# VodLM/vod

Measured on AMD Instinct MI355X. Metric: queries/sec brute-force top-k (10Mx768 fp16), higher is better.
Workload: dtype f16; 1 GPU; 10000000 sections x 768 f16, batch 1024 queries, top-100, exact brute force; rows_per_gpu=10000000, parallelism=single GPU, engine=ranks, recovery_passes=0

## Files before the change

### include/vodhip.h

```cpp
#ifndef VODHIP_H
#define VODHIP_H

#include <stdint.h>

#ifdef __cplusplus
extern "C" {
#endif

#define VODHIP_VERSION 1

enum { VODHIP_F16 = 0, VODHIP_BF16 = 1, VODHIP_F32 = 2 };
#define VODHIP_EXACT_F32 0x100
#define VODHIP_L2 0x200
enum { VODHIP_HOST = 0, VODHIP_DEVICE = 1 };

typedef struct vodhip_index vodhip_index_t;

const char* vodhip_last_error(void);
int vodhip_version(void);

int vodhip_index_create(int device, int64_t dim, int store_dtype ,
                        int64_t capacity_rows, vodhip_index_t** out);
int vodhip_index_destroy(vodhip_index_t* index);

// ... 16 lines not shown
                              int64_t id_base, float* out_scores, int64_t* out_ids, void* stream);
int vodhip_index_search_finish(vodhip_index_t* index, void* stream);

#define VODHIP_MAX_LISTED 8192
int vodhip_index_score_ids(vodhip_index_t* index, const void* queries, int q_dtype, int64_t nq, const int64_t* ids_dev, int64_t m,
                           int64_t id_base, const int32_t* q_labels_dev , int n_per_query,
                           float* out_scores, void* stream);
int vodhip_index_search_ids(vodhip_index_t* index, const void* queries, int q_dtype, int64_t nq, const int64_t* ids_dev, int64_t m,
                            int k, int64_t id_base, const int32_t* q_labels_dev, int n_per_query, float* out_scores,
                            int64_t* out_ids, void* stream);

#define VODHIP_SUM_IDS_TEMP_BYTES (256ll << 20)
int vodhip_index_sum_ids(vodhip_index_t* index, const int64_t* ids_dev, const float* weights_dev, int64_t nq, int64_t m, int64_t id_base,
                         const int32_t* q_labels_dev , int n_per_query, float* out ,
                         void* stream);

int vodhip_index_log_partition(vodhip_index_t* index, const void* queries, int q_dtype, int64_t nq, float beta,
                               const int32_t* q_labels_dev , int n_per_query,
                               float* out_max , float* out_log_rel , void* stream);

#define VODHIP_POSTERIOR_GROUP_ROWS 16384
#define VODHIP_POSTERIOR_TEMP_BYTES (256ll << 20)
int vodhip_index_posterior_mean(vodhip_index_t* index, const void* queries, int q_dtype, int64_t nq, float beta,
                                const int32_t* q_labels_dev , int n_per_query,
                                float* out_max , float* out_log_rel ,
                                float* out_mean , void* stream);

#define VODHIP_SAMPLE_SLACK_TILES 2
int vodhip_index_sample_posterior(vodhip_index_t* index, const void* queries, int q_dtype, int64_t nq, int k, float beta, uint64_t seed,
                                  int64_t query_offset, int64_t id_base, const int32_t* q_labels_dev ,
                                  int n_per_query, float* out_max , float* out_log_rel ,
                                  int64_t* out_ids , float* out_scores, float* out_log_p,
                                  float* out_log_weight , float* out_keys , void* stream);

#define VODHIP_RANK_MAX_LISTED 64
int vodhip_index_count_above(vodhip_index_t* index, const void* queries, int q_dtype, int64_t nq, const float* thresholds_dev,
                             const int64_t* tie_ids_dev , int64_t m, int64_t id_base,
                             const int32_t* q_labels_dev , int n_per_query,
                             int64_t* out_counts , void* stream);
int vodhip_index_rank_ids(vodhip_index_t* index, const void* queries, int q_dtype, int64_t nq, const int64_t* ids_dev, int64_t m,
                          int64_t id_base, const int32_t* q_labels_dev , int n_per_query,
                          int64_t* out_ranks , float* out_scores , void* stream);
int vodhip_index_scan_score_ids(vodhip_index_t* index, const void* queries, int q_dtype, int64_t nq, const int64_t* ids_dev, int64_t m,
                                int64_t id_base, const int32_t* q_labels_dev , int n_per_query,
                                float* out_scores , int32_t* out_rows , void* stream);

int vodhip_index_set_row_labels(vodhip_index_t* index, const int32_t* labels, int64_t n_rows, int location, void* stream);
int vodhip_index_set_query_labels(vodhip_index_t* index, const int32_t* q_labels_dev, int n_per_query);

int vodhip_index_set_param(vodhip_index_t* index, const char* key, int64_t value);
int vodhip_debug_schedule(int64_t ntotal, int k, int64_t nq, int64_t cand_cap, int64_t dense_rows, int64_t sample_div,
                          int64_t growth_x100, int tile, int recovery_pass, int n_cu, int64_t* out, int max_stages);
int vodhip_index_get_stat(const vodhip_index_t* index, const char* key, int64_t* out);
int vodhip_debug_l2_split(float c, int dtype, uint16_t terms[3], float consts[3]);
int vodhip_debug_tile_order(int64_t ntotal, int64_t* perm_mul, int64_t* perm_mod);
int vodhip_debug_read_probe(int which, int64_t* out, int n);

int vodhip_merge_topk(const float* scores, const int64_t* ids, int n_shards, int64_t nq, int k,
                      int k_out, float* out_scores, int64_t* out_ids, void* stream);
int vodhip_merge_topk_strided(const float* scores, int64_t shard_stride_scores, const int64_t* ids,
                              int64_t shard_stride_ids, int n_shards, int64_t nq, int k, int k_out,
                              float* out_scores, int64_t* out_ids, void* stream);

typedef struct vodhip_node_index vodhip_node_index_t;
int vodhip_node_index_create(int n_devices, const int* devices, int64_t dim, int store_dtype, int64_t capacity_rows,
                             vodhip_node_index_t** out);
int vodhip_node_index_destroy(vodhip_node_index_t* index);
int vodhip_node_index_add(vodhip_node_index_t* index, const void* rows, int64_t n_rows, int src_dtype);
int vodhip_node_index_reset(vodhip_node_index_t* index);
int vodhip_node_index_ntotal(const vodhip_node_index_t* index, int64_t* out);
int vodhip_node_index_n_shards(const vodhip_node_index_t* index);
int vodhip_node_index_shard(vodhip_node_index_t* index, int g, vodhip_index_t** shard, int64_t* id_base, int* device);
int vodhip_node_index_set_param(vodhip_node_index_t* index, const char* key, int64_t value);
int vodhip_node_index_peer_access(const vodhip_node_index_t* index, int* out, int n);
int vodhip_node_index_set_row_labels(vodhip_node_index_t* index, const int32_t* labels, int64_t n_rows);
int vodhip_node_index_set_query_labels(vodhip_node_index_t* index, const int32_t* q_labels, int n_per_query, int location);
int vodhip_node_index_search(vodhip_node_index_t* index, const void* queries, int q_dtype, int64_t nq, int k, int location,
                             float* out_scores, int64_t* out_ids, void* stream);
int vodhip_node_index_search_async(vodhip_node_index_t* index, const void* queries, int q_dtype, int64_t nq, int k, int location,
                                   float* out_scores, int64_t* out_ids, void* stream);
int vodhip_node_index_search_finish(vodhip_node_index_t* index);
int vodhip_node_index_score_ids(vodhip_node_index_t* index, const void* queries, int q_dtype, int64_t nq, const int64_t* ids, int64_t m,
                                const int32_t* q_labels, int n_per_query, int location, float* out_scores, void* stream);
int vodhip_node_index_search_ids(vodhip_node_index_t* index, const void* queries, int q_dtype, int64_t nq, const int64_t* ids, int64_t m,
                                 int k, const int32_t* q_labels, int n_per_query, int location, float* out_scores, int64_t* out_ids,
                                 void* stream);
int vodhip_node_index_sum_ids(vodhip_node_index_t* index, const int64_t* ids, const float* weights, int64_t nq, int64_t m,
                              const int32_t* q_labels, int n_per_query, int location, float* out, void* stream);
int vodhip_node_index_log_partition(vodhip_node_index_t* index, const void* queries, int q_dtype, int64_t nq, float beta,
                                    const int32_t* q_labels , int n_per_query,
                                    float* out_max, float* out_log_rel );
int vodhip_node_index_rank_ids(vodhip_node_index_t* index, const void* queries, int q_dtype, int64_t nq, const int64_t* ids, int64_t m,
                               const int32_t* q_labels , int n_per_query,
                               int64_t* out_ranks, float* out_scores );
int vodhip_node_index_count_above(vodhip_node_index_t* index, const void* queries, int q_dtype, int64_t nq, const float* thresholds,
                                  const int64_t* tie_ids , int64_t m,
                                  const int32_t* q_labels , int n_per_query, int64_t* out_counts );
int vodhip_node_index_posterior_mean(vodhip_node_index_t* index, const void* queries, int q_dtype, int64_t nq, float beta,
                                     const int32_t* q_labels , int n_per_query,
                                     float* out_max, float* out_log_rel , float* out_mean );
int vodhip_node_index_sample_posterior(vodhip_node_index_t* index, const void* queries, int q_dtype, int64_t nq, int k, float beta,
                                       uint64_t seed, int64_t query_offset, const int32_t* q_labels , int n_per_query,
                                       float* out_max, float* out_log_rel , int64_t* out_ids, float* out_scores,
                                       float* out_log_p, float* out_log_weight , float* out_keys );
int vodhip_node_index_get_stat(vodhip_node_index_t* index, const char* key, int64_t* out);

// ... 220 lines not shown
```

### vod_amd/_native.py

```python
from __future__ import annotations

import ctypes
import pathlib
import threading

_LIB_NAME = "libvodhip.so"
_lock = threading.Lock()
_lib: ctypes.CDLL | None = None

F16, BF16, F32 = 0, 1, 2
EXACT_F32 = 0x100
L2 = 0x200
METRICS = {"inner_product": 0, "l2": L2}


def metric_flag(metric: str) -> int:
    if metric not in METRICS:
        raise ValueError(f"metric must be one of {sorted(METRICS)}, got {metric!r}")
    return METRICS[metric]
HOST, DEVICE = 0, 1
MAX_K = 2048
MAX_LISTED = 8192
MAX_ENGINES = 4


class NativeLibraryError(RuntimeError):
    """The HIP extension is missing or a native call failed."""


def lib_path() -> pathlib.Path:
    import os

    override = os.environ.get("VODHIP_LIB")
    if override:
        return pathlib.Path(override)
    return pathlib.Path(__file__).resolve().parent / "csrc" / _LIB_NAME


_c = ctypes
_vp, _i64, _i32, _f32p = _c.c_void_p, _c.c_int64, _c.c_int, _c.c_void_p

SIGNATURES: dict[str, tuple] = {
    "vodhip_last_error": (_c.c_char_p, []),
    "vodhip_version": (_i32, []),
    "vodhip_index_create": (_i32, [_i32, _i64, _i32, _i64, _c.POINTER(_vp)]),
    "vodhip_index_destroy": (_i32, [_vp]),
    "vodhip_index_add": (_i32, [_vp, _vp, _i64, _i32, _i32, _vp]),
    "vodhip_index_reset": (_i32, [_vp]),
    "vodhip_index_ntotal": (_i32, [_vp, _c.POINTER(_i64)]),
    "vodhip_index_dim": (_i32, [_vp, _c.POINTER(_i64)]),
    "vodhip_index_capacity": (_i32, [_vp, _c.POINTER(_i64)]),
    "vodhip_index_data": (_i32, [_vp, _c.POINTER(_vp), _c.POINTER(_i64), _c.POINTER(_i32)]),
    "vodhip_index_get_rows": (_i32, [_vp, _i64, _i64, _vp, _i32, _vp]),
    "vodhip_index_data_f32": (_i32, [_vp, _c.POINTER(_vp), _c.POINTER(_i64)]),
    "vodhip_index_get_rows_f32": (_i32, [_vp, _i64, _i64, _vp, _i32, _vp]),
    "vodhip_index_search": (_i32, [_vp, _vp, _i32, _i64, _i32, _i64, _vp, _vp, _vp]),
    "vodhip_index_search_async": (_i32, [_vp, _vp, _i32, _i64, _i32, _i64, _vp, _vp, _vp]),
    "vodhip_index_search_finish": (_i32, [_vp, _vp]),
    "vodhip_index_score_ids": (_i32, [_vp, _vp, _i32, _i64, _vp, _i64, _i64, _vp, _i32, _vp, _vp]),
    "vodhip_index_search_ids": (_i32, [_vp, _vp, _i32, _i64, _vp, _i64, _i32, _i64, _vp, _i32, _vp, _vp, _vp]),
    "vodhip_index_sum_ids": (_i32, [_vp, _vp, _vp, _i64, _i64, _i64, _vp, _i32, _vp, _vp]),
    "vodhip_index_log_partition": (_i32, [_vp, _vp, _i32, _i64, _c.c_float, _vp, _i32, _vp, _vp, _vp]),
    "vodhip_index_posterior_mean": (_i32, [_vp, _vp, _i32, _i64, _c.c_float, _vp, _i32, _vp, _vp, _vp, _vp]),
    "vodhip_index_count_above": (_i32, [_vp, _vp, _i32, _i64, _vp, _vp, _i64, _i64, _vp, _i32, _vp, _vp]),
    "vodhip_index_rank_ids": (_i32, [_vp, _vp, _i32, _i64, _vp, _i64, _i64, _vp, _i32, _vp, _vp, _vp]),
    "vodhip_index_scan_score_ids": (_i32, [_vp, _vp, _i32, _i64, _vp, _i64, _i64, _vp, _i32, _vp, _vp, _vp]),
    "vodhip_index_sample_posterior": (
        _i32, [_vp, _vp, _i32, _i64, _i32, _c.c_float, _c.c_uint64, _i64, _i64, _vp, _i32, _vp, _vp, _vp, _vp, _vp, _vp, _vp, _vp]),
    "vodhip_index_set_row_labels": (_i32, [_vp, _vp, _i64, _i32, _vp]),
    "vodhip_index_set_query_labels": (_i32, [_vp, _vp, _i32]),
    "vodhip_index_set_param": (_i32, [_vp, _c.c_char_p, _i64]),
    "vodhip_debug_schedule": (_i32, [_i64, _i32, _i64, _i64, _i64, _i64, _i64, _i32, _i32, _i32, _c.POINTER(_i64), _i32]),
    "vodhip_index_get_stat": (_i32, [_vp, _c.c_char_p, _c.POINTER(_i64)]),
    "vodhip_debug_l2_split": (_i32, [_c.c_float, _i32, _c.POINTER(_c.c_uint16), _c.POINTER(_c.c_float)]),
    "vodhip_debug_tile_order": (_i32, [_i64, _c.POINTER(_i64), _c.POINTER(_i64)]),
    "vodhip_debug_read_probe": (_i32, [_i32, _c.POINTER(_i64), _i32]),
    "vodhip_node_index_create": (_i32, [_i32, _c.POINTER(_i32), _i64, _i32, _i64, _c.POINTER(_vp)]),
    "vodhip_node_index_destroy": (_i32, [_vp]),
    "vodhip_node_index_add": (_i32, [_vp, _vp, _i64, _i32]),
    "vodhip_node_index_reset": (_i32, [_vp]),
    "vodhip_node_index_ntotal": (_i32, [_vp, _c.POINTER(_i64)]),
    "vodhip_node_index_n_shards": (_i32, [_vp]),
    "vodhip_node_index_shard": (_i32, [_vp, _i32, _c.POINTER(_vp), _c.POINTER(_i64), _c.POINTER(_i32)]),
    "vodhip_node_index_set_param": (_i32, [_vp, _c.c_char_p, _i64]),
    "vodhip_node_index_get_stat": (_i32, [_vp, _c.c_char_p, _c.POINTER(_i64)]),
    "vodhip_node_index_peer_access": (_i32, [_vp, _c.POINTER(_i32), _i32]),
    "vodhip_node_index_set_row_labels": (_i32, [_vp, _vp, _i64]),
    "vodhip_node_index_set_query_labels": (_i32, [_vp, _vp, _i32, _i32]),
    "vodhip_node_index_search": (_i32, [_vp, _vp, _i32, _i64, _i32, _i32, _vp, _vp, _vp]),
    "vodhip_node_index_search_async": (_i32, [_vp, _vp, _i32, _i64, _i32, _i32, _vp, _vp, _vp]),
    "vodhip_node_index_search_finish": (_i32, [_vp]),
    "vodhip_node_index_score_ids": (_i32, [_vp, _vp, _i32, _i64, _vp, _i64, _vp, _i32, _i32, _vp, _vp]),
    "vodhip_node_index_search_ids": (_i32, [_vp, _vp, _i32, _i64, _vp, _i64, _i32, _vp, _i32, _i32, _vp, _vp, _vp]),
    "vodhip_node_index_sum_ids": (_i32, [_vp, _vp, _vp, _i64, _i64, _vp, _i32, _i32, _vp, _vp]),
    "vodhip_node_index_log_partition": (_i32, [_vp, _vp, _i32, _i64, _c.c_float, _vp, _i32, _vp, _vp]),
    "vodhip_node_index_posterior_mean": (_i32, [_vp, _vp, _i32, _i64, _c.c_float, _vp, _i32, _vp, _vp, _vp]),
    "vodhip_node_index_rank_ids": (_i32, [_vp, _vp, _i32, _i64, _vp, _i64, _vp, _i32, _vp, _vp]),
    "vodhip_node_index_count_above": (_i32, [_vp, _vp, _i32, _i64, _vp, _vp, _i64, _vp, _i32, _vp]),
    "vodhip_node_index_sample_posterior": (
        _i32, [_vp, _vp, _i32, _i64, _i32, _c.c_float, _c.c_uint64, _i64, _vp, _i32, _vp, _vp, _vp, _vp, _vp, _vp, _vp]),
    "vodhip_merge_topk": (_i32, [_vp, _vp, _i32, _i64, _i32, _i32, _vp, _vp, _vp]),
    "vodhip_merge_topk_strided": (_i32, [_vp, _i64, _vp, _i64, _i32, _i64, _i32, _i32, _vp, _vp, _vp]),
    "vodhip_merge_hybrid": (
        _i32,
        [_vp, _vp, _i32, _i32, _c.POINTER(_vp), _c.POINTER(_vp), _c.POINTER(_i32), _c.POINTER(_c.c_float), _i64,
         _vp, _vp, _vp, _c.POINTER(_vp), _i32, _vp, _vp, _vp],
    ),
    "vodhip_retrieval_forward": (
        _i32, [_vp, _vp, _i32, _i32, _i64, _i64, _i64, _vp, _vp, _vp, _vp, _vp, _vp, _vp, _vp, _vp, _vp],
    ),
    "vodhip_retrieval_forward_aux": (
        _i32, [_vp, _vp, _i32, _i32, _i64, _i64, _i64, _vp, _vp, _vp, _vp, _i32, _c.c_float, _c.c_float, _c.c_float,
               _vp, _vp, _vp, _vp, _vp, _vp, _vp, _i64, _vp],
    ),
    "vodhip_retrieval_metrics": (_i32, [_vp, _vp, _i64, _i32, _vp, _i32, _vp, _vp, _vp, _i64, _vp]),
    "vodhip_priority_sample": (
        _i32, [_vp, _vp, _vp, _i64, _i32, _i32, _i32, _c.c_float, _i32, _i32, _vp, _vp, _vp, _vp, _vp],
    ),
    "vodhip_priority_sample_merged": (
        _i32, [_vp, _vp, _vp, _i32, _vp, _vp, _i64, _i64, _i32, _i32, _vp, _vp, _i32, _i32, _vp, _i32, _i32, _c.c_float, _i32, _i32,
               _vp, _vp, _vp, _vp, _vp, _vp, _vp, _vp, _vp],
    ),
    "vodhip_priority_sample_proposal": (
        _i32, [_vp, _vp, _vp, _i64, _i32, _i32, _i32, _c.c_float, _i32, _i32, _vp, _vp, _vp, _vp, _vp, _vp, _vp, _vp],
    ),
    "vodhip_priority_sample_merged_proposal": (
# ... 149 lines not shown
```

### vod_amd/csrc/kernels_exact.hip

```cpp
#include <algorithm>

#include "exact_dot.h"
#include "mips_common.h"
#include "wg_sort.h"

namespace vodhip {

namespace {

__device__ __forceinline__ float round_to_store(float f, int store_dtype) {
    float r;
    (void)store_bits(f, store_dtype, &r);
    return r;
}

constexpr int XT = 512;
#ifndef VODHIP_EXACT_NCR
#define VODHIP_EXACT_NCR 4
#endif
constexpr int NCR = VODHIP_EXACT_NCR;

__device__ __forceinline__ void sort_desc_lds(key_t64* keys, int P, int tid) {
    __syncthreads();
    switch (P) {
// ... 299 lines not shown
                default: exact_dot<NCR>(a.plane, a.stride, rows, qs, a.dim_pad, lane, s); break;
            }
            if (lane == 0) {
#pragma unroll
                for (int n = 0; n < NCR; ++n)
                    if (j0 + n < take) kb[KR + j0 + n] = (rows[n] >= 0 && s[n] == s[n]) ? make_key(s[n], (unsigned)rows[n]) : 0ull;
            }
        }
        int P_eff = 64;
        while (P_eff < KR + take) P_eff <<= 1;
        for (int c = KR + take + tid; c < P_eff; c += XT) kb[c] = 0ull;
        sort_desc_lds(kb, P_eff, tid);
        done += take;
    } while (done < n_total);

    const key_t64 kth = kb[k - 1];
    const float s_k = kth ? unflip_f32((unsigned)(kth >> 32)) : -__builtin_inff();
    for (int c = tid; c < k; c += XT) {
        const key_t64 key = kb[c];
        a.out_scores[qo * k + c] = key ? unflip_f32((unsigned)(key >> 32)) : -__builtin_inff();
        a.out_ids[qo * k + c] = key ? a.id_base + (int64_t)(0xFFFFFFFFu - (unsigned)(key & 0xFFFFFFFFull)) : -1;
    }
    __shared__ int need_s;
    if (!cand_mode) {
        if (tid == 0) need_s = 0;
        __syncthreads();
        for (int j = tid; j < a.kx; j += XT)
            if (a.list_i[qo * a.kx + j] >= 0 && a.list_s[qo * a.kx + j] + eps >= s_k) atomicMax(&need_s, j + 1);
        __syncthreads();
    }
    if (tid == 0) {
        if (cand_mode) {
            if (kth) {
                const float t = s_k - eps;
                if (t > a.thr_s[r]) {
                    a.thr_s[r] = t;
                    a.thr_key[r] = (key_t64)flip_f32(t) << 32;
                }
            }
            a.cnt[(size_t)r * CNT_STRIDE] = 0;
            if (lost) {
                atomicOr(a.flag_word, 1u);
                if (a.flag_q) a.flag_q[r] = 1u;
            }
        } else {
            a.eps[qo] = eps;
            const bool full = a.list_i[qo * a.kx + a.kx - 1] >= 0;
            const bool complete = !full || (a.list_s[qo * a.kx + a.kx - 1] + eps < s_k);
            a.flag_q[qo] = complete ? 0u : 1u;
            if (!complete) atomicOr(a.flag_word, 1u);
            if ((unsigned)need_s > __hip_atomic_load(a.flag_word + 1, __ATOMIC_RELAXED, __HIP_MEMORY_SCOPE_AGENT)) atomicMax(a.flag_word + 1, (unsigned)need_s);
        }
    }
}

hipError_t launch_exact_rescore(const ExactArgs& a, int64_t nq, hipStream_t stream) {
    if (nq <= 0) return hipSuccess;
    const int bytes = (int)((size_t)a.dim_pad * sizeof(float) + (size_t)a.P * (sizeof(key_t64) + sizeof(int)));
    if (hipError_t e = allow_dynamic_lds((const void*)exact_rescore_kernel, bytes); e != hipSuccess) return e;
    hipLaunchKernelGGL(exact_rescore_kernel, dim3((unsigned)nq), dim3(XT), bytes, stream, a);
    return hipGetLastError();
}

}
```

### vod_amd/csrc/kernels_l2.hip

```cpp
#include "../../include/vodhip.h"
#include "l2_bias.h"

extern "C" int vodhip_debug_l2_split(float c, int dtype, uint16_t terms[3], float consts[3]) {
    if ((dtype != VODHIP_F16 && dtype != VODHIP_BF16) || !terms || !consts) return -1;
    uint16_t bits[3];
    vodhip::l2_query_consts(dtype, consts, bits);
    return vodhip::l2_split(c, dtype, terms);
}

#if defined(__HIP__)
#include "mips_common.h"

namespace vodhip {

namespace {

template <int DT>
__device__ __forceinline__ float l2_from_bits(uint16_t b) {
    if constexpr (DT == 0) return (float)__builtin_bit_cast(_Float16, b);
    else return __uint_as_float((unsigned int)b << 16);
}

__device__ __forceinline__ float l2_wave_sum(float v) {
#pragma unroll
// ... 10 lines not shown
    uint16_t* x = rows + row * stride;
    float acc = 0.f;
    for (int c0 = lane * 8; c0 < dim; c0 += 64 * 8) {
        const uint4 w = *(const uint4*)(x + c0);
        const unsigned int u[4] = {w.x, w.y, w.z, w.w};
#pragma unroll
        for (int e = 0; e < 8; ++e) {
            const float v = l2_from_bits<DT>((uint16_t)(u[e >> 1] >> ((e & 1) * 16)));
            if (c0 + e < dim) acc = fmaf(v, v, acc);
        }
    }
    const float n2 = l2_wave_sum(acc);
    if (lane == 0) {
        uint16_t t[3];
        if (l2_split(-0.5f * n2, DT, t)) atomicAdd(saturated, 1u);
        x[dim] = t[0];
        x[dim + 1] = t[1];
        x[dim + 2] = t[2];
    }
}

template <int DT>
__global__ void __launch_bounds__(256) l2_stage_queries_kernel(const void* __restrict__ q_src, int q_dtype, int64_t nq, int dim,
                                                               uint16_t* __restrict__ staged, float* __restrict__ qn) {
    const int lane = threadIdx.x & 63;
    const int64_t row = (int64_t)blockIdx.x * 4 + (threadIdx.x >> 6);
    if (row >= nq) return;
    uint16_t* out = staged + row * (int64_t)(dim + L2_BIAS_COLS);
    float acc = 0.f;
    for (int c0 = lane * 8; c0 < dim; c0 += 64 * 8) {
        for (int e = 0; e < 8 && c0 + e < dim; ++e) {
            const int64_t at = row * dim + c0 + e;
            float f;
            if (q_dtype == 2) f = ((const float*)q_src)[at];
            else if (q_dtype == 0) f = (float)(((const _Float16*)q_src)[at]);
            else f = (float)(((const __bf16*)q_src)[at]);
            float v;
            out[c0 + e] = store_bits(f, DT, &v);
            acc = fmaf(v, v, acc);
        }
    }
    const float n2 = l2_wave_sum(acc);
    if (lane == 0) {
        float a[3];
        uint16_t bits[3];
        l2_query_consts(DT, a, bits);
        out[dim] = bits[0];
        out[dim + 1] = bits[1];
        out[dim + 2] = bits[2];
        qn[row] = n2;
    }
}

__global__ void __launch_bounds__(256) l2_finish_kernel(const float* __restrict__ sim, const float* __restrict__ qn, int64_t nq, int k, float* __restrict__ dist) {
    const int64_t i = (int64_t)blockIdx.x * blockDim.x + threadIdx.x;
    if (i >= nq * k) return;
    const float s = sim[i];
    float d = __builtin_inff();
    if (s != -__builtin_inff()) d = fmaxf(0.f, qn[i / k] - 2.f * s);
    dist[i] = d;
}

}

hipError_t launch_l2_bias(void* rows, int store_dtype, int64_t n_rows, int64_t dim, int64_t stride, unsigned int* saturated,
                          hipStream_t stream) {
    if (n_rows == 0) return hipSuccess;
    if (dim + L2_BIAS_COLS > stride || stride % 64 != 0 || dim > (1ll << 30)) return hipErrorInvalidValue;
    const unsigned blocks = (unsigned)((n_rows + 3) / 4);
    if (store_dtype == 0)
        hipLaunchKernelGGL(l2_bias_kernel<0>, dim3(blocks), dim3(256), 0, stream, (uint16_t*)rows, n_rows, (int)dim, stride, saturated);
    else
        hipLaunchKernelGGL(l2_bias_kernel<1>, dim3(blocks), dim3(256), 0, stream, (uint16_t*)rows, n_rows, (int)dim, stride, saturated);
    return hipGetLastError();
}

hipError_t launch_l2_stage_queries(const void* q_src, int q_dtype, int64_t nq, int64_t dim, int store_dtype, void* staged, float* qn,
                                   hipStream_t stream) {
    if (nq == 0) return hipSuccess;
    if (dim > (1ll << 30)) return hipErrorInvalidValue;
    const unsigned blocks = (unsigned)((nq + 3) / 4);
    if (store_dtype == 0)
        hipLaunchKernelGGL(l2_stage_queries_kernel<0>, dim3(blocks), dim3(256), 0, stream, q_src, q_dtype, nq, (int)dim, (uint16_t*)staged, qn);
    else
        hipLaunchKernelGGL(l2_stage_queries_kernel<1>, dim3(blocks), dim3(256), 0, stream, q_src, q_dtype, nq, (int)dim, (uint16_t*)staged, qn);
    return hipGetLastError();
}

hipError_t launch_l2_finish(const float* sim, const float* qn, int64_t nq, int k, float* dist, hipStream_t stream) {
    if (nq == 0) return hipSuccess;
    const int64_t n = nq * k;
    hipLaunchKernelGGL(l2_finish_kernel, dim3((unsigned)((n + 255) / 256)), dim3(256), 0, stream, sim, qn, nq, k, dist);
    return hipGetLastError();
}

}
#endif
```

### vod_amd/csrc/kernels_mips.hip

```cpp
#include "mips_common.h"
#include "wg_sort.h"

#include <algorithm>
#include <cstdlib>
#include <map>
#include <mutex>
#include <utility>
#include <type_traits>

namespace vodhip {

enum : int { MODE_FILTER = 0, MODE_DENSE = 1, MODE_GMAX = 2 };

template <int DT, int BM, int BN, int WM, int WN, int NSTAGE, int MODE, bool SUBSET = false>
__global__ __launch_bounds__(WM* WN * 64, (WM * WN * 64 * ((160 * 1024) / (NSTAGE * (BM + BN) * 128))) / 256 >= 2 ? 2 : 1)
void mips_filter_kernel(
    const uint16_t* __restrict__ X, const uint16_t* __restrict__ Q, int dim_pad, int row_begin, int row_end,
    int n_xtiles, int n_qtiles, int nq, const float* __restrict__ thr_s, const key_t64* __restrict__ thr_key,
    key_t64* __restrict__ cand, unsigned int* __restrict__ cnt, int cap, unsigned int* __restrict__ overflow, FilterExtra ex) {
    constexpr int BK = 64;
    constexpr int NWAVES = WM * WN;
    constexpr int TM = BM / WM, TN = BN / WN;
    constexpr int MI = TM / 32, NJ = TN / 32;
    constexpr int ROW_BYTES = BK * 2;
    constexpr int RPI = 8;
    constexpr int KK = BK / 16;
    constexpr int A_BYTES = BM * ROW_BYTES, B_BYTES = BN * ROW_BYTES;
    constexpr int STAGE_BYTES = A_BYTES + B_BYTES;
    constexpr int NA = BM / RPI / NWAVES;
    constexpr int NB = BN / RPI / NWAVES;
    constexpr int G = NA + NB;
    static_assert(BM % (RPI * NWAVES) == 0 && BN % (RPI * NWAVES) == 0, "tile/wave mismatch");
    static_assert(NSTAGE >= 2 && NSTAGE <= 3, "ring depth");

    extern __shared__ __attribute__((aligned(16))) char smem[];

    const int bid = blockIdx.x;
    const int xcd = bid & 7, jj = bid >> 3;
    const int qt = jj % n_qtiles;
    const int xt = (jj / n_qtiles) * 8 + xcd;
    if (xt >= n_xtiles) return;

    const int tid = threadIdx.x;
    const int lane = tid & 63;
    const int wave = __builtin_amdgcn_readfirstlane(tid >> 6);
    const int wm = wave / WN, wn = wave % WN;

    const int x0 = MODE == MODE_FILTER ? filter_tile_row0(ex, row_begin, xt, BM) : row_begin + xt * BM;
    const int q0 = qt * BN;

    const int st_row = lane >> 3, st_slot = lane & 7;
    const char* a_src[NA];
    const char* b_src[NB];
#pragma unroll
    for (int t = 0; t < NA; ++t) {
        const int r = (wave * NA + t) * RPI + st_row;
        const int c = st_slot ^ ((r >> 1) & 7);
        size_t grow = (size_t)(x0 + r);
        if constexpr (MODE == MODE_GMAX) {
            const int bb = r & 31;
            const int grp_in_tile = ((r / TM) * MI + (r % TM) / 32) * 2 + ((bb >> 2) & 1);
            const int idx = (bb >> 3) * 4 + (bb & 3);
            grow = ((size_t)idx * (size_t)ex.sample_groups + (size_t)xt * (BM / 16) + grp_in_tile) * (size_t)ex.sample_rstride + (size_t)ex.sample_offset;
        }
        a_src[t] = (const char*)X + (grow * dim_pad + c * 8) * 2;
    }
#pragma unroll
    for (int t = 0; t < NB; ++t) {
        const int r = (wave * NB + t) * RPI + st_row;
        const int c = st_slot ^ ((r >> 1) & 7);
        b_src[t] = (const char*)Q + ((size_t)(q0 + r) * dim_pad + c * 8) * 2;
    }
    auto stage_part = [&](int ks, int part, int nparts) {
        char* sa = smem + (ks % NSTAGE) * STAGE_BYTES;
        char* sb = sa + A_BYTES;
        const int kbyte = ks * ROW_BYTES;
#pragma unroll
        for (int u = 0; u < G; ++u) {
            if ((u * nparts) / G != part) continue;
            if (u < NA)
                glds16(a_src[u] + kbyte, sa + (wave * NA + u) * RPI * ROW_BYTES);
            else
                glds16(b_src[u - NA] + kbyte, sb + (wave * NB + (u - NA)) * RPI * ROW_BYTES);
        }
    };

    const int fr = lane & 31, fh = lane >> 5;
    const int swz = (fr >> 1) & 7;
    const int a_row_off = (wm * TM + fr) * ROW_BYTES;
    const int b_row_off = A_BYTES + (wn * TN + fr) * ROW_BYTES;

    f32x16 acc[MI][NJ];
#pragma unroll
    for (int i = 0; i < MI; ++i)
// ... 55 lines not shown
    }
    for (; t < nk; ++t) {
        if (NSTAGE >= 3 && nk - 1 - t >= 1) wait_vmcnt<(NSTAGE >= 3 ? 1 : 0) * G>();
        else wait_vmcnt<0>();
        __builtin_amdgcn_s_barrier();
        kslice(t, std::false_type{});
    }

#pragma unroll
    for (int j = 0; j < NJ; ++j) {
        const int q = q0 + wn * TN + j * 32 + fr;
        const bool q_ok = q < nq;
#pragma unroll
        for (int i = 0; i < MI; ++i) {
            const int rbase = x0 + wm * TM + i * 32 + 4 * fh;
            if constexpr (MODE == MODE_DENSE) {
                if (q_ok) {
#pragma unroll
                    for (int r = 0; r < 16; ++r) {
                        const int row = rbase + (r & 3) + 8 * (r >> 2);
                        const float s = acc[i][j][r];
                        if (row < row_end) {
                            const key_t64 key = (s == s) ? make_key(s, (unsigned)row) : 0ull;
                            cand[(size_t)q * cap + (row - row_begin)] = key;
                        }
                    }
                    if constexpr (SUBSET) {
#pragma unroll 1
                        for (int r = 0; r < 16; ++r) {
                            const int row = rbase + (r & 3) + 8 * (r >> 2);
                            if (row < row_end && !subset_allows(ex, q, row)) cand[(size_t)q * cap + (row - row_begin)] = 0ull;
                        }
                    }
                }
            } else {
                float m = acc[i][j][0];
#pragma unroll
                for (int r = 1; r < 16; ++r) m = fmaxf(m, acc[i][j][r]);
                if constexpr (MODE == MODE_GMAX) {
                    const int slot = xt * (BM / 16) + (wm * MI + i) * 2 + fh;
                    if (q_ok) cand[(size_t)q * cap + slot] = (m == m) ? make_key(m, (unsigned)slot) : 0ull;
                } else {
                    const bool hit = m >= thr[j];
                    if (__any(hit)) {
                        if (hit)
                            append_survivors<16, SUBSET>(
                                thr[j], q, row_end, [&](int r) { return acc[i][j][r]; },
                                [&](int r) { return rbase + (r & 3) + 8 * (r >> 2); }, thr_key, cand, cnt, cap, overflow, ex);
                    }
                }
            }
        }
    }
}

constexpr int WSTG_CAP = 256;
constexpr int WSTG_FLUSH = 176;
constexpr int WSTG_BYTES = 8 * WSTG_CAP * 12;
template <int DT, int MODE, bool SUBSET, bool STAGGER>
__global__ __launch_bounds__(512, 2) void mips_filter16p_kernel(
    const uint16_t* __restrict__ X, const uint16_t* __restrict__ Q, int dim_pad, int row_begin, int row_end,
    int n_xtiles, int n_qtiles, int nq, const float* __restrict__ thr_s, const key_t64* __restrict__ thr_key,
    key_t64* __restrict__ cand, unsigned int* __restrict__ cnt, int cap, unsigned int* __restrict__ overflow, FilterExtra ex) {
    static_assert(MODE == MODE_FILTER || MODE == MODE_GMAX, "dense chunks run on mips_filter_kernel");
    constexpr int BM = 256, BN = 256, WN = 4, NWAVES = 8, BK = 64, NSTAGE = 2;
    constexpr int TM = 128, TN = 64;
    constexpr int MB = TM / 16, NB16 = TN / 16;
    constexpr int ROW_BYTES = BK * 2, RPI = 8;
    constexpr int A_BYTES = BM * ROW_BYTES, STAGE_BYTES = (BM + BN) * ROW_BYTES;
    constexpr int NA = BM / RPI / NWAVES, NBI = BN / RPI / NWAVES, G = NA + NBI;

    extern __shared__ __attribute__((aligned(16))) char smem[];
    const int bid = blockIdx.x;
    const int xcd = bid & 7, jj = bid >> 3;
    const int qt = jj % n_qtiles;
    const int xt0 = (jj / n_qtiles) * 8 + xcd;
    const int xt_step = (int)gridDim.x / n_qtiles;
    if (xt0 >= n_xtiles) return;
    const int n_my = (n_xtiles - 1 - xt0) / xt_step + 1;
    const int tid = threadIdx.x;
    const int lane = tid & 63;
    const int wave = __builtin_amdgcn_readfirstlane(tid >> 6);
    const int wm = wave / WN, wn = wave % WN;
    const int q0 = qt * BN;
    const int nk = dim_pad / BK;
    const size_t tile_rows_stride = MODE == MODE_GMAX ? (size_t)8 * (size_t)ex.sample_rstride : (size_t)BM;
    size_t tile_step_bytes = (size_t)xt_step * tile_rows_stride * dim_pad * 2;
#ifdef VODHIP_ABLATION
    const bool abl_l2hot = (ex.flags & (1 << 8)) != 0;
    const bool abl_dma_early = (ex.flags & (2 << 8)) != 0;
    const bool abl_prio = (ex.flags & (4 << 8)) != 0;
    const bool abl_nosurv = (ex.flags & (8 << 8)) != 0;
    const bool abl_corpus_nt = (ex.flags & (16 << 8)) != 0;
    const bool abl_corpus_sc0 = (ex.flags & (32 << 8)) != 0;
    const bool abl_blocked = (ex.flags & (64 << 8)) != 0;
    const bool abl_q0 = (ex.flags & (128 << 8)) != 0;
    if (abl_l2hot) tile_step_bytes = 0;
    if (abl_prio && wave >= NWAVES / 2) __builtin_amdgcn_s_setprio(1);
#else
    constexpr bool abl_l2hot = false, abl_dma_early = false, abl_nosurv = false, abl_blocked = false, abl_q0 = false;
#endif

    const int st_row = lane >> 3, st_slot = lane & 7;
    const char* a_src[NA];
    const char* b_src[NBI];
#pragma unroll
    for (int t = 0; t < NA; ++t) {
        const int r = (wave * NA + t) * RPI + st_row;
        size_t grow = (size_t)filter_tile_row0(ex, row_begin, abl_l2hot ? (xt0 & 15) : xt0, BM) + r;
        if constexpr (MODE == MODE_GMAX) {
            const int grp_in_tile = (r >> 7) * 4 + ((r >> 2) & 3);
            const int idx = ((r >> 4) & 7) * 4 + (r & 3);
            grow = ((size_t)idx * (size_t)ex.sample_groups + (size_t)xt0 * 8 + grp_in_tile) * (size_t)ex.sample_rstride + (size_t)ex.sample_offset;
        }
        a_src[t] = (const char*)X + (grow * dim_pad + (st_slot ^ ((r >> 1) & 7)) * 8) * 2;
        if (abl_blocked)
            a_src[t] = (const char*)X + ((size_t)row_begin + (size_t)xt0 * BM) * dim_pad * 2 + (size_t)r * ROW_BYTES + (st_slot ^ ((r >> 1) & 7)) * 16;
    }
#pragma unroll
    for (int t = 0; t < NBI; ++t) {
        const int r = (wave * NBI + t) * RPI + st_row;
        b_src[t] = (const char*)Q + ((size_t)((abl_q0 ? 0 : q0) + r) * dim_pad + (st_slot ^ ((r >> 1) & 7)) * 8) * 2;
    }
    const bool corpus_nt = (ex.flags & FILTER_FLAG_CORPUS_NT) != 0;
    auto stage_part = [&](int slot, int kbyte, int part, int nparts) {
        char* sa = smem + slot * STAGE_BYTES;
        char* sb = sa + A_BYTES;
#pragma unroll
        for (int u = 0; u < G; ++u) {
            if ((u * nparts) / G != part) continue;
            if (u < NA) {
// ... 148 lines not shown
        ++g;
    };
    Frags fp;
    bool pre_b = false;
    int kbyte_b = 0;
    auto slice_b_head = [&](int it, int t) {
        wait_vmcnt<0>();
        __builtin_amdgcn_s_barrier();
        next_fetch(it, t, pre_b, kbyte_b);
        if (pre_b) stage_part((g + 1) & 1, kbyte_b, 0, 2);
    };
    auto slice_b_body = [&](auto first_tag) {
        constexpr bool FIRST = decltype(first_tag)::value;
        const char* base = smem + (g & 1) * STAGE_BYTES;
        __builtin_amdgcn_sched_barrier(0);
        Frags f;
        read_b(base, 0, f);
        read_a(base, 0, f, 0, 8);
        if (pre_b) stage_part((g + 1) & 1, kbyte_b, 1, 2);
        __builtin_amdgcn_sched_barrier(0);
        mma(f, 0, 8, FIRST);
        __builtin_amdgcn_sched_barrier(0);
        read_b(base, 1, fp);
        read_a(base, 1, fp, 0, 8);
        asm volatile("s_waitcnt lgkmcnt(0)" ::: "memory");
        __builtin_amdgcn_sched_barrier(0);
        ++g;
    };
    if (!STAGGER || wave < NWAVES / 2) {
        for (int it = 0; it < n_my; ++it) {
            slice_a(it, 0, std::true_type{});
            for (int t = 1; t < nk; ++t) slice_a(it, t, std::false_type{});
            epilogue(xt0 + it * xt_step, tile_row0(it));
        }
    } else {
        for (int it = 0; it <= n_my; ++it) {
            if (it < n_my) slice_b_head(it, 0);
            if (it > 0) {
                mma(fp, 0, 8, false);
                __builtin_amdgcn_sched_barrier(0);
                epilogue(xt0 + (it - 1) * xt_step, tile_row0(it - 1));
            }
            if (it < n_my) {
                slice_b_body(std::true_type{});
                for (int t = 1; t < nk; ++t) {
                    slice_b_head(it, t);
                    mma(fp, 0, 8, false);
                    slice_b_body(std::false_type{});
                }
            }
        }
    }
    if constexpr (MODE == MODE_FILTER) wl.flush(out);
}

__device__ __forceinline__ void bitonic_sort_desc_lds(key_t64* keys, int P, int tid) {
    constexpr int CE_UNROLL = 4;
    const int half = P >> 1;
    for (int size = 2; size <= P; size <<= 1) {
        for (int stride = size >> 1; stride > 0; stride >>= 1) {
            __syncthreads();
            for (int t0 = tid; t0 < half; t0 += 256 * CE_UNROLL) {
                key_t64 a[CE_UNROLL], b[CE_UNROLL];
                int pos[CE_UNROLL];
#pragma unroll
                for (int u = 0; u < CE_UNROLL; ++u) {
                    const int t = t0 + u * 256;
                    pos[u] = 2 * t - (t & (stride - 1));
                    if (t < half) {
                        a[u] = keys[pos[u]];
                        b[u] = keys[pos[u] + stride];
                    }
                }
#pragma unroll
                for (int u = 0; u < CE_UNROLL; ++u) {
                    const int t = t0 + u * 256;
                    if (t < half) {
                        const bool desc = (pos[u] & size) == 0;
                        if ((a[u] < b[u]) == desc) {
                            keys[pos[u]] = b[u];
                            keys[pos[u] + stride] = a[u];
                        }
                    }
                }
            }
        }
    }
    __syncthreads();
}

constexpr int SEL_HIST_INTS = 544;

template <typename Op>
__device__ __forceinline__ int wave_scan_dpp(int v, int identity, Op op) {
    v = op(v, __builtin_amdgcn_update_dpp(identity, v, 0x111, 0xf, 0xf, false));
    v = op(v, __builtin_amdgcn_update_dpp(identity, v, 0x112, 0xf, 0xf, false));
    v = op(v, __builtin_amdgcn_update_dpp(identity, v, 0x114, 0xf, 0xf, false));
    v = op(v, __builtin_amdgcn_update_dpp(identity, v, 0x118, 0xf, 0xf, false));
    v = op(v, __builtin_amdgcn_update_dpp(identity, v, 0x142, 0xa, 0xf, false));
    v = op(v, __builtin_amdgcn_update_dpp(identity, v, 0x143, 0xc, 0xf, false));
    return v;
}
#ifdef VODHIP_ABLATION
__device__ long long g_probe_select[256];
#endif
#define RSEL_PROBE(i) VODHIP_PROBE(g_probe_select, ppb + (i))
// ... 63 lines not shown
                    hist[514] = hh[j];
                }
        }
        __syncthreads();
        if (pass < 4) RSEL_PROBE(2 + 2 * pass);
        const int digit = hist[512];
        rank = hist[513];
        const int in_bin = hist[514];
        prefix |= (key_t64)digit << sh;
        mask |= dmask << sh;
        hi_bit = sh - 1;
        if (in_bin == 1 && hi_bit >= 0) {
#pragma unroll
            for (int u = 0; u < KPT; ++u) {
                const key_t64 e = mine[u];
                if (e != 0ull && (e & mask) == prefix) {
                    hist[515] = (int)(unsigned)(e & 0xFFFFFFFFull);
                    hist[516] = (int)(unsigned)(e >> 32);
                }
            }
            __syncthreads();
            return ((key_t64)(unsigned)hist[516] << 32) | (key_t64)(unsigned)hist[515];
        }
    }
    return prefix;
}

__device__ __forceinline__ void sort_front_desc(key_t64* keys, int kp, int tid) {
    __syncthreads();
    if (kp <= 512) {
        if (tid < 64) {
            switch (kp) {
                case 64: wave_sort_regs<1, true>(keys, tid); break;
                case 128: wave_sort_regs<2, true>(keys, tid); break;
                case 256: wave_sort_regs<4, true>(keys, tid); break;
                default: wave_sort_regs<8, true>(keys, tid); break;
            }
        }
        __syncthreads();
    } else if (!wg_sort_lds_256<true>(keys, kp, tid)) {
        bitonic_sort_desc_lds(keys, kp, tid);
    }
}

enum : int { SELECT_FINAL = 1, SELECT_THRESHOLD_ONLY = 2 };
#define SEL_PROBE(i) VODHIP_PROBE(g_probe_select, pb + (i))
template <int KPT>
__global__ __launch_bounds__(256) void mips_select_kernel(key_t64* __restrict__ topk, int kp, int k,
                                                          const key_t64* __restrict__ cand,
                                                          unsigned int* __restrict__ cnt, int cap, int dense_n,
                                                          float* __restrict__ thr_s, key_t64* __restrict__ thr_key,
                                                          unsigned int* __restrict__ overflow, unsigned int* __restrict__ ovf_q, int flags,
                                                          int64_t id_base, float* __restrict__ out_scores,
                                                          int64_t* __restrict__ out_ids, const int* __restrict__ q_map) {
    extern __shared__ __attribute__((aligned(16))) char smem[];
    int* hist = (int*)smem;
    key_t64* front = (key_t64*)(hist + SEL_HIST_INTS);
    const int q = blockIdx.x;
    const int tid = threadIdx.x;
    const bool final_sort = (flags & SELECT_FINAL) != 0;
    const bool thr_only = (flags & SELECT_THRESHOLD_ONLY) != 0;
    [[maybe_unused]] const int pb = final_sort ? 0 : thr_only ? 8 : 16;
    SEL_PROBE(0);
    key_t64 mine[KPT];
    const key_t64* cq = cand + (size_t)q * cap;
#pragma unroll
    for (int u = 0; u < KPT; ++u) {
        const int i = tid + u * 256;
        if (i < kp) mine[u] = thr_only ? 0ull : topk[(size_t)q * kp + i];
        else mine[u] = (i - kp) < cap ? cq[i - kp] : 0ull;
    }
    unsigned n = dense_n >= 0 ? (unsigned)dense_n : cnt[(size_t)q * CNT_STRIDE];
    if (n > (unsigned)cap) {
        if (tid == 0) {
            atomicOr(overflow, 1u);
            if (ovf_q) ovf_q[q] = 1u;
        }
        n = cap;
    }
    const int room = KPT * 256 - kp;
    int done = 0;
    key_t64 kth = 0;
    do {
        const int take = min((int)n - done, room);
        const int total = kp + take;
        if (done > 0) {
#pragma unroll
            for (int u = 0; u < KPT; ++u) {
                const int i = tid + u * 256;
                mine[u] = i < kp ? front[i] : (i < total ? cq[done + (i - kp)] : 0ull);
            }
        } else {
#pragma unroll
            for (int u = 0; u < KPT; ++u)
                if (tid + u * 256 >= total) mine[u] = 0ull;
        }
        if (tid == 0) hist[517] = 0;
        SEL_PROBE(1);
        kth = radix_select_kth_regs<KPT>(mine, k, hist, tid, 24 + 10 * (pb >> 3));
        SEL_PROBE(2);
        done += take;
        if (!thr_only || done < (int)n) {
            unsigned long long keep[KPT];
            int n_wave = 0;
#pragma unroll
            for (int u = 0; u < KPT; ++u) {
                keep[u] = __ballot(mine[u] >= kth && mine[u] != 0ull);
                n_wave += __builtin_popcountll(keep[u]);
            }
            int base = 0;
            if ((tid & 63) == 0 && n_wave) base = atomicAdd(&hist[517], n_wave);
            base = __builtin_amdgcn_readfirstlane(base);
            const unsigned long long below = (1ull << (tid & 63)) - 1ull;
#pragma unroll
            for (int u = 0; u < KPT; ++u) {
                const int at = base + __builtin_popcountll(keep[u] & below);
                if (((keep[u] >> (tid & 63)) & 1ull) && at < kp) front[at] = mine[u];
                base += __builtin_popcountll(keep[u]);
            }
            __syncthreads();
            const int n_kept = min(hist[517], kp);
            for (int i = n_kept + tid; i < kp; i += 256) front[i] = 0ull;
            __syncthreads();
        }
    } while (done < (int)n);
    SEL_PROBE(3);
    if (final_sort) {
        sort_front_desc(front, kp, tid);
        kth = front[k - 1];
    }
    SEL_PROBE(4);
    if (!thr_only)
        for (int i = tid; i < kp; i += 256) topk[(size_t)q * kp + i] = front[i];
    if (out_scores != nullptr) {
        const size_t qo = q_map ? (size_t)q_map[q] : (size_t)q;
        for (int c = tid; c < k; c += 256) {
            const key_t64 key = front[c];
            out_scores[qo * k + c] = key ? unflip_f32((unsigned)(key >> 32)) : -__builtin_inff();
            out_ids[qo * k + c] = key ? id_base + (int64_t)(0xFFFFFFFFu - (unsigned)(key & 0xFFFFFFFFu)) : -1;
        }
    }
    if (tid == 0) {
        if (thr_only) kth &= 0xFFFFFFFF00000000ull;
        const key_t64 old = thr_key[q];
        if (kth > old) {
            thr_key[q] = kth;
            thr_s[q] = unflip_f32((unsigned)(kth >> 32));
        }
        cnt[(size_t)q * CNT_STRIDE] = 0;
    }
    SEL_PROBE(5);
    if (tid == 0 && q == 0) {
        [[maybe_unused]] const long long nn = (long long)n;
#ifdef VODHIP_ABLATION
        g_probe_select[2 * (pb + 6)] = nn;
        g_probe_select[2 * (pb + 6) + 1] = 1;
#endif
    }
}

__global__ void mips_output_kernel(const key_t64* __restrict__ topk, int kp, int k, int64_t nq, int64_t id_base,
                                   float* __restrict__ out_scores, int64_t* __restrict__ out_ids) {
    const int64_t i = (int64_t)blockIdx.x * blockDim.x + threadIdx.x;
    if (i >= nq * k) return;
    const int64_t q = i / k;
    const int c = (int)(i % k);
    const key_t64 key = topk[q * kp + c];
    if (key == 0) {
        out_scores[i] = -__builtin_inff();
        out_ids[i] = -1;
    } else {
        out_scores[i] = unflip_f32((unsigned)(key >> 32));
        out_ids[i] = id_base + (int64_t)(0xFFFFFFFFu - (unsigned)(key & 0xFFFFFFFFu));
    }
}

template <int SRC, int DST>
__global__ void convert_rows_kernel(const void* __restrict__ src, int64_t n_rows, int64_t dim, uint16_t* __restrict__ dst,
                                    int64_t dst_stride) {
    const int64_t chunks_per_row = dst_stride / 8;
    const int64_t i = (int64_t)blockIdx.x * blockDim.x + threadIdx.x;
    if (i >= n_rows * chunks_per_row) return;
    const int64_t row = i / chunks_per_row;
    const int64_t c0 = (i % chunks_per_row) * 8;
    uint16_t out[8];
#pragma unroll
    for (int e = 0; e < 8; ++e) {
        const int64_t c = c0 + e;
        uint16_t v = 0;
        if (c < dim) {
            float f;
            if constexpr (SRC == 2) {
                f = ((const float*)src)[row * dim + c];
            } else if constexpr (SRC == 0) {
                f = (float)(((const _Float16*)src)[row * dim + c]);
            } else {
                f = (float)(((const __bf16*)src)[row * dim + c]);
            }
            float rounded;
            v = store_bits(f, DST, &rounded);
        }
        out[e] = v;
    }
    *(uint4*)(dst + row * dst_stride + c0) = *(const uint4*)out;
}

hipError_t launch_convert_rows(const void* src, int src_dtype, int64_t n_rows, int64_t dim, void* dst, int dst_dtype,
                               int64_t dst_stride, hipStream_t stream) {
    if (n_rows == 0) return hipSuccess;
    const int64_t total = n_rows * (dst_stride / 8);
    const int threads = 256;
// ... 8 lines not shown
    VOD_CONV(0, 0) VOD_CONV(1, 0) VOD_CONV(2, 0) VOD_CONV(0, 1) VOD_CONV(1, 1) VOD_CONV(2, 1)
#undef VOD_CONV
    return hipErrorInvalidValue;
}

__global__ void mips_prepare_kernel(const void* __restrict__ q_src, int q_dtype, int64_t nq, int64_t dim,
                                    uint16_t* __restrict__ q_pad, int store_dtype, int64_t nq_pad, int64_t dim_pad,
                                    key_t64* __restrict__ topk, int64_t n_topk, unsigned int* __restrict__ cnt,
                                    float* __restrict__ thr_s, key_t64* __restrict__ thr_key,
                                    unsigned int* __restrict__ overflow, unsigned int* __restrict__ ovf_q, int clear_overflow,
                                    const float* __restrict__ seed_scores, const int64_t* __restrict__ seed_ids, int k,
                                    const int* __restrict__ q_map, const float* __restrict__ seed_margin) {
    const int64_t i = (int64_t)blockIdx.x * blockDim.x + threadIdx.x;
    const int64_t chunks_per_row = dim_pad / 8;
    if (i < nq_pad * chunks_per_row) {
        const int64_t row = i / chunks_per_row;
        const int64_t c0 = (i % chunks_per_row) * 8;
        uint16_t out[8];
#pragma unroll
        for (int e = 0; e < 8; ++e) {
            const int64_t c = c0 + e;
            uint16_t v = 0;
            if (row < nq && c < dim) {
                const int64_t srow = q_map ? (int64_t)q_map[row] : row;
                float f;
                if (q_dtype == 2) f = ((const float*)q_src)[srow * dim + c];
                else if (q_dtype == 0) f = (float)(((const _Float16*)q_src)[srow * dim + c]);
                else f = (float)(((const __bf16*)q_src)[srow * dim + c]);
                float rounded;
                v = store_bits(f, store_dtype, &rounded);
            }
            out[e] = v;
        }
        *(uint4*)(q_pad + row * dim_pad + c0) = *(const uint4*)out;
    }
    if (i < n_topk) topk[i] = 0;
    if (i < nq_pad) {
        cnt[i * CNT_STRIDE] = 0;
        float ts = -__builtin_inff();
        key_t64 tk = 0;
        const int64_t srow = (q_map && i < nq) ? (int64_t)q_map[i] : i;
        if (ovf_q != nullptr && i < nq) ovf_q[i] = 0u;
        if (seed_scores != nullptr && i < nq && seed_ids[srow * k + (k - 1)] >= 0) {
            float s = seed_scores[srow * k + (k - 1)];
            if (seed_margin != nullptr) s -= seed_margin[srow];
            if (s == s) {
                ts = s;
                tk = (key_t64)flip_f32(s) << 32;
            }
        }
        thr_s[i] = ts;
        thr_key[i] = tk;
    }
    if (i == 0 && clear_overflow) {
        overflow[0] = 0u;
        overflow[1] = 0u;
        overflow[2] = 0u;
        overflow[3] = 0u;
    }
}

hipError_t launch_search_prepare(const SearchWorkspace& ws, const void* q_src, int q_dtype, int64_t nq, int64_t dim,
                                 int store_dtype, int64_t nq_pad, int64_t dim_pad, bool clear_overflow,
                                 const float* seed_scores, const int64_t* seed_ids, int k, const int* q_map, hipStream_t stream,
                                 const float* seed_margin) {
    const int64_t n_topk = nq_pad * ws.kp;
    const int64_t n = std::max(n_topk, nq_pad * (dim_pad / 8));
    const int threads = 256;
    const unsigned blocks = (unsigned)((n + threads - 1) / threads);
    hipLaunchKernelGGL(mips_prepare_kernel, dim3(blocks), dim3(threads), 0, stream, q_src, q_dtype, nq, dim,
                       (uint16_t*)ws.q_pad, store_dtype, nq_pad, dim_pad, ws.topk, n_topk, ws.cnt, ws.thr_s, ws.thr_key,
                       ws.overflow, ws.ovf_q, clear_overflow ? 1 : 0, seed_scores, seed_ids, k, q_map, seed_margin);
    return hipGetLastError();
}

hipError_t allow_dynamic_lds(const void* kernel, int bytes) {
    static std::mutex mu;
    static std::map<std::pair<int, const void*>, int> granted;
    int dev = 0;
    hipError_t e = hipGetDevice(&dev);
    if (e != hipSuccess) return e;
    std::lock_guard<std::mutex> lock(mu);
    auto it = granted.find({dev, kernel});
    if (it != granted.end() && it->second >= bytes) return hipSuccess;
    e = hipFuncSetAttribute(kernel, hipFuncAttributeMaxDynamicSharedMemorySize, bytes);
    if (e == hipSuccess) granted[{dev, kernel}] = bytes;
    return e;
}

namespace {

struct FilterLaunch {
    const void* store;
    const void* q_pad;
    int64_t dim_pad, row_begin, row_end, nq, nq_pad;
    int n_xtiles;
    const SearchWorkspace* ws;
    hipStream_t stream;
};

template <int DT, int BM, int BN, int WM, int WN, int NSTAGE, int MODE, bool SUBSET>
hipError_t launch_generic(const FilterLaunch& L) {
    const int n_qtiles = (int)(L.nq_pad / BN);
    const unsigned grid = (unsigned)((L.n_xtiles + 7) / 8) * 8u * (unsigned)n_qtiles;
    constexpr int threads = WM * WN * 64;
    constexpr size_t lds = (size_t)NSTAGE * (BM + BN) * 128;
    auto kern = mips_filter_kernel<DT, BM, BN, WM, WN, NSTAGE, MODE, SUBSET>;
// ... 30 lines not shown
    if (hipError_t e = allow_dynamic_lds((const void*)kern, (int)lds); e != hipSuccess) return e;
    const SearchWorkspace& ws = *L.ws;
    hipLaunchKernelGGL(kern, dim3((unsigned)grid), dim3(512), lds, L.stream, (const uint16_t*)L.store, (const uint16_t*)L.q_pad,
                       (int)L.dim_pad, (int)L.row_begin, (int)L.row_end, L.n_xtiles, n_qtiles, (int)L.nq, ws.thr_s, ws.thr_key,
                       ws.cand, ws.cnt, (int)ws.cap, ws.overflow, ws.extra);
    return hipGetLastError();
}

template <int DT, bool STAGGER>
hipError_t launch_persistent_mode(const FilterLaunch& L, int mode, bool subset) {
    constexpr FilterGeometry G = geometry(STAGGER ? FilterKernel::Staggered : FilterKernel::Persistent);
    static_assert(G.rows == 256 && G.cols == 256 && G.group_rows == 32 && G.persistent, "the planner's geometry of mips_filter16p_kernel");
    if (mode == MODE_DENSE) return hipErrorInvalidValue;
    if (mode == MODE_GMAX) return launch_persistent<DT, MODE_GMAX, false, STAGGER>(L);
    return subset ? launch_persistent<DT, MODE_FILTER, true, STAGGER>(L) : launch_persistent<DT, MODE_FILTER, false, STAGGER>(L);
}

template <int DT>
hipError_t launch_filter_dt(FilterKernel kernel, int mode, bool subset, const FilterLaunch& L) {
    switch (kernel) {
        case FilterKernel::Generic128: return launch_generic_mode<DT, FilterKernel::Generic128, 128, 128, 2, 2, 2>(L, mode, subset);
        case FilterKernel::Generic256x64: return launch_generic_mode<DT, FilterKernel::Generic256x64, 256, 64, 4, 1, 3>(L, mode, subset);
        case FilterKernel::Generic256x128: return launch_generic_mode<DT, FilterKernel::Generic256x128, 256, 128, 4, 2, 3>(L, mode, subset);
        case FilterKernel::Persistent: return launch_persistent_mode<DT, false>(L, mode, subset);
        case FilterKernel::Staggered: return launch_persistent_mode<DT, true>(L, mode, subset);
        default: return hipErrorInvalidValue;
    }
}

}

hipError_t launch_filter(int store_dtype, FilterKernel kernel, int mode, const void* store, const void* q_pad, int64_t dim_pad,
                         int64_t row_begin, int64_t row_end, int64_t n_sample_tiles, int64_t nq, int64_t nq_pad,
                         const SearchWorkspace& ws, hipStream_t stream, FilterStageFn experiment) {
    if (mode != MODE_GMAX && row_end <= row_begin) return hipSuccess;
    if (mode == MODE_GMAX && n_sample_tiles <= 0) return hipSuccess;
    if (experiment && mode == MODE_FILTER) return experiment(store_dtype, store, q_pad, dim_pad, row_begin, row_end, nq, nq_pad, ws, stream);
    if (kernel == FilterKernel::EightPhase)
        return mode == MODE_FILTER ? launch_filter_8phase(store_dtype, 7, true, store, q_pad, dim_pad, row_begin, row_end, nq, nq_pad, ws, stream)
                                   : hipErrorInvalidValue;
    const int bm = geometry(kernel).rows;
    int n_xtiles = mode == MODE_GMAX ? (int)n_sample_tiles : (int)((row_end - row_begin + bm - 1) / bm);
    if (mode == MODE_FILTER && ws.extra.perm_mod > 0) {
        n_xtiles = (int)((row_end - row_begin + 255) / 256) * (256 / bm);
        row_end = ws.extra.row_bound;
    }
    FilterLaunch L{store, q_pad, dim_pad, row_begin, row_end, nq, nq_pad, n_xtiles, &ws, stream};
    const bool subset = ws.extra.row_label != nullptr;
    return store_dtype == 0 ? launch_filter_dt<0>(kernel, mode, subset, L) : launch_filter_dt<1>(kernel, mode, subset, L);
}

template <int KPT>
static hipError_t launch_select_kpt(const SearchWorkspace& ws, int64_t nq, int k, int64_t dense_n, int flags, hipStream_t stream,
                                    int64_t id_base, float* out_scores, int64_t* out_ids, const int* q_map) {
    const size_t lds = SEL_HIST_INTS * sizeof(int) + (size_t)ws.kp * sizeof(key_t64);
    const bool final_sort = (flags & SELECT_FINAL) != 0;
    hipLaunchKernelGGL(mips_select_kernel<KPT>, dim3((unsigned)nq), dim3(256), lds, stream, ws.topk, (int)ws.kp, k, ws.cand,
                       ws.cnt, (int)ws.cap, (int)dense_n, ws.thr_s, ws.thr_key, ws.overflow, ws.ovf_q, flags, id_base,
                       final_sort ? out_scores : nullptr, final_sort ? out_ids : nullptr, q_map);
    return hipGetLastError();
}

hipError_t launch_select(const SearchWorkspace& ws, int64_t nq, int k, int64_t dense_n, int flags, hipStream_t stream,
                         int64_t id_base, float* out_scores, int64_t* out_ids, const int* q_map) {
    int sb = 2048;
    while (sb < 2 * ws.kp) sb <<= 1;
    while (dense_n > sb - ws.kp && sb < 8192) sb <<= 1;
    switch (sb) {
        case 2048: return launch_select_kpt<8>(ws, nq, k, dense_n, flags, stream, id_base, out_scores, out_ids, q_map);
        case 4096: return launch_select_kpt<16>(ws, nq, k, dense_n, flags, stream, id_base, out_scores, out_ids, q_map);
        default: return launch_select_kpt<32>(ws, nq, k, dense_n, flags, stream, id_base, out_scores, out_ids, q_map);
    }
}

hipError_t launch_output(const SearchWorkspace& ws, int64_t nq, int k, int64_t id_base, float* out_scores,
                         int64_t* out_ids, hipStream_t stream) {
    const int64_t total = nq * k;
    if (total == 0) return hipSuccess;
    const unsigned blocks = (unsigned)((total + 255) / 256);
    hipLaunchKernelGGL(mips_output_kernel, dim3(blocks), dim3(256), 0, stream, ws.topk, (int)ws.kp, k, nq, id_base,
                       out_scores, out_ids);
    return hipGetLastError();
}

__device__ __forceinline__ bool pair_before(float sa, int64_t ia, float sb, int64_t ib) {
    const bool va = ia >= 0, vb = ib >= 0;
    if (va != vb) return va;
    if (!va) return false;
    if (sa != sb) return sa > sb;
    return ia < ib;
}

__device__ __forceinline__ void merge_ce(float* ssc, int64_t* sid, int a, int b) {
    const float sa = ssc[a], sb = ssc[b];
    const int64_t ia = sid[a], ib = sid[b];
    if (pair_before(sb, ib, sa, ia)) {
        ssc[a] = sb;
        ssc[b] = sa;
        sid[a] = ib;
        sid[b] = ia;
    }
}

__global__ __launch_bounds__(256) void merge_topk_kernel(const float* __restrict__ scores, const int64_t* __restrict__ ids,
                                                         int64_t stride_s, int64_t stride_i, int n_shards, int64_t nq, int k, int k_out,
                                                         int L, int S2, int flat, float* __restrict__ out_scores,
                                                         int64_t* __restrict__ out_ids) {
    extern __shared__ __attribute__((aligned(16))) char smem[];
    const int P = S2 * L;
    int64_t* sid = (int64_t*)smem;
    float* ssc = (float*)(smem + (size_t)P * 8);
    int* s_flag = (int*)(smem + (size_t)P * 12);
    const int64_t q = blockIdx.x;
    const int tid = threadIdx.x;
    const int lmask = L - 1, lshift = 31 - __builtin_clz(L);
    if (tid == 0) *s_flag = 0;
    for (int i = tid; i < P; i += 256) {
        const int t = flat ? i / k : i >> lshift, c = flat ? i % k : i & lmask;
        float s = -__builtin_inff();
        int64_t id = -1;
        if (t < n_shards && c < k) {
            s = scores[(int64_t)t * stride_s + q * k + c];
            id = ids[(int64_t)t * stride_i + q * k + c];
            if (id < 0 || s != s) {
// ... 88 lines not shown
```

### vod_amd/csrc/kernels_mips_8phase.hip

```cpp
#include <hip/hip_runtime.h>

#include <type_traits>

#include "mips_common.h"

namespace vodhip {

namespace {
constexpr int P8_HALF = 128 * 128;
constexpr int P8_OPERANDS = 8 * P8_HALF;
constexpr int P8_WL_CAP = 256;
constexpr int P8_WL_FLUSH = 176;
constexpr int P8_TRANSPOSE_MAX_LANES = 2;
constexpr int P8_XPOSE = 8 * 2 * 32 * 4;
constexpr int P8_DRAIN_RECORDS = 112;
constexpr int P8_SC1 = 16;
static_assert(P8_DRAIN_RECORDS % 8 == 0 && P8_DRAIN_RECORDS * 132 + 256 <= P8_OPERANDS / 8, "drain staging");
constexpr int P8_LDS = P8_OPERANDS + 8 * P8_WL_CAP * 12 + P8_XPOSE;
static_assert(P8_LDS <= 160 * 1024, "LDS budget");
}

template <int DT, bool SUBSET, bool KEEPB0, int LEAD = 7>
__global__ __launch_bounds__(512, 2) void mips_filter8ph_kernel(
    const uint16_t* __restrict__ X, const uint16_t* __restrict__ Q, int dim_pad, int row_begin, int row_end, int n_xtiles,
    int n_qtiles, int nq, const float* __restrict__ thr_s, const key_t64* __restrict__ thr_key, key_t64* __restrict__ cand,
    unsigned int* __restrict__ cnt, int cap, unsigned int* __restrict__ overflow, FilterExtra ex, float* __restrict__ ring, int ring_cap) {
    constexpr int BM = 256, BN = 256, WN = 4, NWAVES = 8, TM = 128, TN = 64, MB = TM / 16, NB16 = TN / 16, ROW_BYTES = 128;
    extern __shared__ __attribute__((aligned(16))) char smem[];
    const int bid = blockIdx.x;
    const int xcd = bid & 7, jj = bid >> 3;
    const int qt = jj % n_qtiles;
    const int xt0 = (jj / n_qtiles) * 8 + xcd;
    const int xt_step = (int)gridDim.x / n_qtiles;
    if (xt0 >= n_xtiles) return;
    const int n_my = (n_xtiles - 1 - xt0) / xt_step + 1;
    const int tid = threadIdx.x;
    const int lane = tid & 63;
    const int wave = __builtin_amdgcn_readfirstlane(tid >> 6);
    const int wm = wave / WN, wn = wave % WN;
    const int q0 = qt * BN;
    const int nk = dim_pad / 64;
    const size_t row_stride = (size_t)dim_pad * 2;

    const int st_row = lane >> 3, st_slot = lane & 7;
    int super_cur = ex.perm_mod > 0 ? filter_tile_row0(ex, row_begin, xt0, BM) / BM : 0;
    int super_epi = super_cur;
    const int perm_inc = ex.perm_mod > 0 ? (int)(((unsigned long long)xt_step * (unsigned long long)ex.perm_mul) % (unsigned long long)ex.perm_mod) : 0;
    const char* a_src[2];
    const char* b_src[2];
#pragma unroll
    for (int u = 0; u < 2; ++u) {
        const int sw = (u * 4 + (st_row >> 1)) & 7;
        const int arow = (wave >> 2) * 128 + (wave & 3) * 16 + u * 8 + st_row;
        const int brow = (wave >> 1) * 64 + (wave & 1) * 16 + u * 8 + st_row;
        a_src[u] = (const char*)X + ((size_t)filter_tile_row0(ex, row_begin, xt0, BM) + arow) * row_stride + ((st_slot ^ sw) << 4);
#ifdef VODHIP_ABLATION
        const int q0_stage = (ex.flags & (128 << 8)) ? 0 : q0;
#else
        const int q0_stage = q0;
#endif
        b_src[u] = (const char*)Q + (size_t)(q0_stage + brow) * row_stride + ((st_slot ^ sw) << 4);
    }
    const size_t a_half_step = 64 * row_stride, b_half_step = 32 * row_stride;
    const size_t tile_step_bytes = (size_t)xt_step * BM * row_stride;

    const bool corpus_nt = (ex.flags & FILTER_FLAG_CORPUS_NT) != 0;
    int s_t = 0, s_it = 0, s_par = 0;
    int issued = 0;
    bool s_active = n_my > 0;
    auto stage = [&](auto kind_tag) {
        constexpr int KIND = decltype(kind_tag)::value;
        if (s_active) {
            char* dst = smem + (s_par * 4 + KIND) * P8_HALF + wave * 16 * ROW_BYTES;
            const int kbyte = s_t * ROW_BYTES;
            if constexpr (KIND == 0 || KIND == 2) {
                const size_t off = (KIND == 2 ? a_half_step : 0) + kbyte;
                if (corpus_nt) {
                    glds16_aux<2>(a_src[0] + off, dst);
                    glds16_aux<2>(a_src[1] + off, dst + 8 * ROW_BYTES);
                } else {
                    glds16(a_src[0] + off, dst);
                    glds16(a_src[1] + off, dst + 8 * ROW_BYTES);
                }
            } else if constexpr (KIND == 1) {
                glds16(b_src[0] + b_half_step + kbyte, dst);
                glds16(b_src[1] + b_half_step + kbyte, dst + 8 * ROW_BYTES);
            } else {
                glds16(b_src[0] + kbyte, dst);
                glds16(b_src[1] + kbyte, dst + 8 * ROW_BYTES);
            }
            ++issued;
            if constexpr (KIND == 3) {
                s_par ^= 1;
                if (++s_t == nk) {
                    s_t = 0;
                    ++s_it;
                    if (s_it < n_my) {
                        long long step = (long long)tile_step_bytes;
                        if (ex.perm_mod > 0) {
                            int nxt = super_cur + perm_inc;
                            if (nxt >= ex.perm_mod) nxt -= ex.perm_mod;
                            step = (long long)(nxt - super_cur) * (long long)BM * (long long)row_stride;
                            super_cur = nxt;
                        }
                        a_src[0] += step;
                        a_src[1] += step;
                    } else {
                        s_active = false;
                    }
                }
            }
        }
    };
    using K0 = std::integral_constant<int, 0>;
    using K1 = std::integral_constant<int, 1>;
    using K2 = std::integral_constant<int, 2>;
    using K3 = std::integral_constant<int, 3>;

    const int fr = lane & 15, fq = lane >> 4;
    const int swz = (fr >> 1) & 7;

    float thr[NB16];
#pragma unroll
    for (int j = 0; j < NB16; ++j) {
        const int q = q0 + wn * TN + j * 16 + fr;
        thr[j] = q < nq ? thr_s[q] : __builtin_inff();
    }
#pragma unroll
    for (int j = 0; j < NB16; ++j) asm volatile("" : "+v"(thr[j]));
    wait_vmcnt<0>();

    WaveSurvivorList<P8_WL_CAP, SUBSET> wl(smem + P8_OPERANDS, NWAVES, wave);
    const SurvivorOut out{thr_key, cand, cnt, cap, overflow, ex};
    auto wl_append = [&](bool p, key_t64 key, int q) { if (wl.append(p, key, q, out)) wait_vmcnt<0>(); };
    auto wl_flush = [&]() { wl.flush(out); wait_vmcnt<0>(); };
    float* const xpose = (float*)(smem + P8_OPERANDS + NWAVES * P8_WL_CAP * 12) + wave * 64;
    const size_t ring_wave = (size_t)bid * NWAVES + wave;
    float* const ring_w = ring + ring_wave * ring_cap * 32;
    unsigned* const ring_meta = (unsigned*)(ring + (size_t)gridDim.x * NWAVES * ring_cap * 32) + ring_wave * ring_cap;
    int ring_n = 0;
    int ring_fallbacks = 0;

    f32x4 acc[MB][NB16];
    u32x4 fa[4], fb[2], fa1[4], fb1[2];
    u32x4 fc[2], fc1[2];
#ifdef P8_KNOBS
    const bool knob_no_stagger = (ex.flags & (1 << 8)) != 0, knob_no_prio = (ex.flags & (2 << 8)) != 0;
#else
    constexpr bool knob_no_stagger = false, knob_no_prio = false;
#endif

    auto read_a = [&](const char* half) {
        const char* base = half + (wm * 64 + fr) * ROW_BYTES;
        const int s0 = ((0 + fq) ^ swz) << 4, s1 = ((4 + fq) ^ swz) << 4;
#pragma unroll
        for (int i = 0; i < 4; ++i) {
            fa[i] = *(const u32x4*)(base + i * 16 * ROW_BYTES + s0);
            fa1[i] = *(const u32x4*)(base + i * 16 * ROW_BYTES + s1);
        }
    };
    auto read_b = [&](const char* half) {
        const char* base = half + (wn * 32 + fr) * ROW_BYTES;
        const int s0 = ((0 + fq) ^ swz) << 4, s1 = ((4 + fq) ^ swz) << 4;
#pragma unroll
        for (int j = 0; j < 2; ++j) {
            fb[j] = *(const u32x4*)(base + j * 16 * ROW_BYTES + s0);
            fb1[j] = *(const u32x4*)(base + j * 16 * ROW_BYTES + s1);
        }
    };
    auto read_b1 = [&](const char* half) {
        const char* base = half + (wn * 32 + fr) * ROW_BYTES;
        const int s0 = ((0 + fq) ^ swz) << 4, s1 = ((4 + fq) ^ swz) << 4;
#pragma unroll
        for (int j = 0; j < 2; ++j) {
            if constexpr (KEEPB0) {
                fc[j] = *(const u32x4*)(base + j * 16 * ROW_BYTES + s0);
                fc1[j] = *(const u32x4*)(base + j * 16 * ROW_BYTES + s1);
            } else {
                fb[j] = *(const u32x4*)(base + j * 16 * ROW_BYTES + s0);
                fb1[j] = *(const u32x4*)(base + j * 16 * ROW_BYTES + s1);
            }
        }
    };
// ... 198 lines not shown
        if (ex.perm_mod > 0) {
            int nxt = super_epi + perm_inc;
            if (nxt >= ex.perm_mod) nxt -= ex.perm_mod;
            super_epi = nxt;
        }
    }
    if (wm == 0 && !knob_no_stagger) __builtin_amdgcn_s_barrier();

#ifndef P8_ABL_NO_DRAIN
    if (ring_n > 0) {
        wait_vmcnt<0>();
        if (fq == 0) {
#pragma unroll
            for (int j = 0; j < NB16; ++j) xpose[j * 16 + fr] = thr[j];
        }
        wave_lds_exchange();
        char* const stage_w = smem + wave * (P8_OPERANDS / NWAVES);
        const float* const sums = (const float*)stage_w;
        const unsigned* const meta = (const unsigned*)(stage_w + P8_DRAIN_RECORDS * 128);
        const int half = lane >> 5, t = lane & 31;
        for (int r0 = 0; r0 < ring_n; r0 += P8_DRAIN_RECORDS) {
#pragma unroll
            for (int i = 0; i < P8_DRAIN_RECORDS / 8; ++i) {
                const int r = min(r0 + i * 8 + (lane >> 3), ring_n - 1);
                __builtin_amdgcn_global_load_lds((const VOD_AS1 void*)(ring_w + (size_t)r * 32 + (lane & 7) * 4),
                                                 (VOD_AS3 void*)(stage_w + i * 1024), 16, 0, P8_SC1);
            }
#pragma unroll
            for (int i = 0; i < (P8_DRAIN_RECORDS + 63) / 64; ++i) {
                const int r = min(r0 + i * 64 + lane, ring_n - 1);
                __builtin_amdgcn_global_load_lds((const VOD_AS1 void*)(ring_meta + r), (VOD_AS3 void*)(stage_w + P8_DRAIN_RECORDS * 128 + i * 256),
                                                 4, 0, P8_SC1);
            }
            wait_vmcnt<0>();
            const int nr = min(ring_n - r0, P8_DRAIN_RECORDS);
            for (int r4 = 0; r4 < nr; r4 += 4) {
                if (wl.n > P8_WL_CAP - 128) wl_flush();
                const int r = r4 + half;
#pragma unroll
                for (int u = 0; u < 4; u += 2) {
                    const float v = sums[(r + u) * 32 + t];
                    const unsigned m = meta[r + u];
                    const int src = (int)(m & 63u), jb = (int)((m >> 6) & 3u), x0 = (int)(m & ~255u);
                    const int q_src = q0 + wn * TN + jb * 16 + (src & 15);
                    const int rw = x0 + wm * TM + 4 * (src >> 4) + (t >> 2) * 16 + (t & 3);
                    wl_append(r + u < nr && v >= xpose[jb * 16 + (src & 15)] && rw < row_end, make_key(v, (unsigned)rw), q_src);
                }
            }
        }
    }
#endif
    wl_flush();
    if (ring_fallbacks > 0 && lane == 0) atomicAdd(overflow + 3, (unsigned)ring_fallbacks);
}

template <bool KEEPB0, int LEAD = 7>
static hipError_t launch_8phase(int store_dtype, const void* store, const void* q_pad, int64_t dim_pad, int64_t row_begin, int64_t row_end, int n_xtiles,
                                   int64_t nq, int64_t nq_pad, const SearchWorkspace& ws, hipStream_t stream) {
    const bool subset = ws.extra.row_label != nullptr;
    const int n_qtiles = (int)(nq_pad / 256);
    const int n_cu = ws.n_cu > 0 ? ws.n_cu : 256;
    const int unit = 8 * n_qtiles;
    const int total = ((n_xtiles + 7) / 8) * unit;
    int grid = (n_cu / unit) * unit;
    if (grid < unit) grid = unit;
    if (grid > total) grid = total;
    const int ring_cap = ws.ring ? (int)std::min<int64_t>(ws.ring_cap, ws.ring_floats / ((int64_t)grid * 8 * 33)) : 0;
    auto launch = [&](auto kern) -> hipError_t {
        if (hipError_t e = allow_dynamic_lds((const void*)kern, P8_LDS); e != hipSuccess) return e;
        hipLaunchKernelGGL(kern, dim3((unsigned)grid), dim3(512), P8_LDS, stream, (const uint16_t*)store, (const uint16_t*)q_pad, (int)dim_pad,
                           (int)row_begin, (int)row_end, n_xtiles, n_qtiles, (int)nq, ws.thr_s, ws.thr_key, ws.cand, ws.cnt, (int)ws.cap,
                           ws.overflow, ws.extra, ws.ring, ring_cap);
        return hipGetLastError();
    };
    if constexpr (LEAD != 7)
        return store_dtype == 0 ? launch(mips_filter8ph_kernel<0, false, KEEPB0, LEAD>) : launch(mips_filter8ph_kernel<1, false, KEEPB0, LEAD>);
    else if (subset) return store_dtype == 0 ? launch(mips_filter8ph_kernel<0, true, KEEPB0>) : launch(mips_filter8ph_kernel<1, true, KEEPB0>);
    else return store_dtype == 0 ? launch(mips_filter8ph_kernel<0, false, KEEPB0>) : launch(mips_filter8ph_kernel<1, false, KEEPB0>);
}

hipError_t launch_filter_8phase(int store_dtype, int lead, bool keep_b0, const void* store, const void* q_pad, int64_t dim_pad, int64_t row_begin,
                                int64_t row_end, int64_t nq, int64_t nq_pad, const SearchWorkspace& ws, hipStream_t stream) {
    constexpr FilterGeometry G = geometry(FilterKernel::EightPhase);
    static_assert(G.rows == 256 && G.cols == 256 && G.persistent, "the planner's geometry of mips_filter8ph_kernel");
    int n_xtiles = (int)((row_end - row_begin + 255) / 256);
    if (ws.extra.perm_mod > 0) row_end = ws.extra.row_bound;
#ifdef VODHIP_EXPERIMENTS
    if (lead == 6) return launch_8phase<true, 6>(store_dtype, store, q_pad, dim_pad, row_begin, row_end, n_xtiles, nq, nq_pad, ws, stream);
    if (lead == 5) return launch_8phase<true, 5>(store_dtype, store, q_pad, dim_pad, row_begin, row_end, n_xtiles, nq, nq_pad, ws, stream);
    if (!keep_b0) return launch_8phase<false>(store_dtype, store, q_pad, dim_pad, row_begin, row_end, n_xtiles, nq, nq_pad, ws, stream);
#endif
    (void)lead;
    (void)keep_b0;
    return launch_8phase<true>(store_dtype, store, q_pad, dim_pad, row_begin, row_end, n_xtiles, nq, nq_pad, ws, stream);
}

}
```

### vod_amd/csrc/mips_common.h

```cpp
#pragma once
#include "vodhip_internal.h"

namespace vodhip {

typedef _Float16 f16x8 __attribute__((ext_vector_type(8)));
typedef __bf16 bf16x8 __attribute__((ext_vector_type(8)));
typedef float f32x16 __attribute__((ext_vector_type(16)));
typedef float f32x4 __attribute__((ext_vector_type(4)));
typedef unsigned int u32x4 __attribute__((ext_vector_type(4)));

#define VOD_AS1 __attribute__((address_space(1)))
#define VOD_AS3 __attribute__((address_space(3)))

__device__ __forceinline__ unsigned int flip_f32(float s) {
    unsigned int u = __float_as_uint(s + 0.0f);
    return (u & 0x80000000u) ? ~u : (u | 0x80000000u);
}
__device__ __forceinline__ float unflip_f32(unsigned int u) {
    return __uint_as_float((u & 0x80000000u) ? (u & 0x7fffffffu) : ~u);
}
__device__ __forceinline__ key_t64 make_key(float s, unsigned int local_row) {
    return ((key_t64)flip_f32(s) << 32) | (key_t64)(0xFFFFFFFFu - local_row);
}

// ... 21 lines not shown
        return __builtin_amdgcn_mfma_f32_32x32x16_f16(__builtin_bit_cast(f16x8, a), __builtin_bit_cast(f16x8, b), c, 0, 0, 0);
    } else {
        return __builtin_amdgcn_mfma_f32_32x32x16_bf16(__builtin_bit_cast(bf16x8, a), __builtin_bit_cast(bf16x8, b), c, 0, 0, 0);
    }
}
template <int DT>
__device__ __forceinline__ f32x4 mfma16(u32x4 a, u32x4 b, f32x4 c) {
    if constexpr (DT == 0) {
        return __builtin_amdgcn_mfma_f32_16x16x32_f16(__builtin_bit_cast(f16x8, a), __builtin_bit_cast(f16x8, b), c, 0, 0, 0);
    } else {
        return __builtin_amdgcn_mfma_f32_16x16x32_bf16(__builtin_bit_cast(bf16x8, a), __builtin_bit_cast(bf16x8, b), c, 0, 0, 0);
    }
}

__device__ __forceinline__ void glds16(const void* gsrc, void* lds_dst) {
    __builtin_amdgcn_global_load_lds((const VOD_AS1 void*)gsrc, (VOD_AS3 void*)lds_dst, 16, 0, 0);
}

template <int AUX>
__device__ __forceinline__ void glds16_aux(const void* gsrc, void* lds_dst) {
    __builtin_amdgcn_global_load_lds((const VOD_AS1 void*)gsrc, (VOD_AS3 void*)lds_dst, 16, 0, AUX);
}

__device__ __forceinline__ float vmax3(float a, float b, float c) {
    float r;
    asm("v_max3_f32 %0, %1, %2, %3" : "=v"(r) : "v"(a), "v"(b), "v"(c));
    return r;
}
__device__ __forceinline__ float fmaxf_raw(float a, float b) {
    float r;
    asm("v_max_f32 %0, %1, %2" : "=v"(r) : "v"(a), "v"(b));
    return r;
}

template <int N>
__device__ __forceinline__ void wait_vmcnt() {
    if constexpr (N == 0) asm volatile("s_waitcnt vmcnt(0)" ::: "memory");
    else if constexpr (N == 2) asm volatile("s_waitcnt vmcnt(2)" ::: "memory");
    else if constexpr (N == 4) asm volatile("s_waitcnt vmcnt(4)" ::: "memory");
    else if constexpr (N == 5) asm volatile("s_waitcnt vmcnt(5)" ::: "memory");
    else if constexpr (N == 6) asm volatile("s_waitcnt vmcnt(6)" ::: "memory");
    else if constexpr (N == 8) asm volatile("s_waitcnt vmcnt(8)" ::: "memory");
    else if constexpr (N == 10) asm volatile("s_waitcnt vmcnt(10)" ::: "memory");
    else if constexpr (N == 12) asm volatile("s_waitcnt vmcnt(12)" ::: "memory");
    else static_assert(N == 0, "add the literal");
}

__device__ __forceinline__ int filter_tile_row0(const FilterExtra& ex, int row_begin, int xt, int BM) {
    if (ex.perm_mod <= 0) return row_begin + xt * BM;
    const int per = 256 / BM;
    const unsigned long long pos = (unsigned long long)(row_begin / 256 + xt / per);
    const int super = (int)((pos * (unsigned long long)ex.perm_mul) % (unsigned long long)ex.perm_mod);
    return super * 256 + (xt % per) * BM;
}

__device__ __forceinline__ bool subset_allows(const FilterExtra& ex, int q, int row) {
    if (ex.row_label == nullptr) return true;
    const int lab = ex.row_label[row];
    const int qq = ex.q_map ? ex.q_map[q] : q;
    bool any = false, ok = false;
#pragma unroll 1
    for (int s = 0; s < ex.n_qlab; ++s) {
        const int ql = ex.q_label[(size_t)qq * ex.n_qlab + s];
        any |= ql != -1;
        ok |= ql == lab;
    }
    return ok || !any;
}

struct SurvivorOut {
    const key_t64* thr_key;
    key_t64* cand;
    unsigned int* cnt;
    int cap;
    unsigned int* overflow;
    const FilterExtra& ex;
};

template <bool SUBSET>
__device__ __forceinline__ void emit_candidate(key_t64 key, int q, const SurvivorOut& out) {
    bool ok = key > out.thr_key[q];
    if constexpr (SUBSET) ok = ok && subset_allows(out.ex, q, (int)(0xFFFFFFFFu - (unsigned)key));
    if (ok) {
        const unsigned slot = atomicAdd(&out.cnt[(size_t)q * CNT_STRIDE], 1u);
        if (slot < (unsigned)out.cap)
            out.cand[(size_t)q * out.cap + slot] = key;
        else
            atomicOr(out.overflow, 1u);
    }
}

template <int CAP, bool SUBSET>
struct WaveSurvivorList {
    key_t64* const key;
    int* const q;
    const int lane = (int)threadIdx.x & 63;
    int n = 0;

    __device__ WaveSurvivorList(char* area, int n_lists, int list)
        : key((key_t64*)area + list * CAP), q((int*)(area + n_lists * CAP * 8) + list * CAP) {}

    __device__ bool append(bool p, key_t64 k, int qq, const SurvivorOut& out) {
        const unsigned long long bal = __ballot(p);
        if (bal == 0ull) return false;
        const int pos = n + (int)__builtin_amdgcn_mbcnt_hi((unsigned)(bal >> 32), __builtin_amdgcn_mbcnt_lo((unsigned)bal, 0u));
        bool direct = false;
// ... 116 lines not shown
```

### vod_amd/csrc/vodhip_api.hip

```cpp
#include "../../include/vodhip.h"

#include <algorithm>
#include <atomic>
#include <cmath>
#include <cstdarg>
#include <cstdio>
#include <cstdint>
#include <cstring>
#include <string>
#include <deque>
#include <initializer_list>
#include <mutex>
#include <thread>
#include <vector>

#include "l2_bias.h"
#include "partition_fold.h"
#include "sample_fold.h"
#include "rank_fold.h"
#include "search_plan.h"
#include "vodhip_internal.h"

using namespace vodhip;

namespace {

thread_local std::string g_last_error;

int fail(const char* fmt, ...) {
    char buf[1024];
    va_list ap;
    va_start(ap, fmt);
    vsnprintf(buf, sizeof(buf), fmt, ap);
    va_end(ap);
    g_last_error = buf;
    return -1;
}

}

namespace vodhip {
void set_last_error(const char* msg) { g_last_error = msg ? msg : ""; }
}

namespace {

#define HIP_OK(expr)                                                                            \
    do {                                                                                        \
        hipError_t _e = (expr);                                                                 \
        if (_e != hipSuccess) {                                                                 \
            (void)hipGetLastError();  \
            return fail("%s failed: %s (%s:%d)", #expr, hipGetErrorString(_e), __FILE__, __LINE__); \
        }                                                                                       \
    } while (0)

constexpr int64_t STAGE_BYTES = 64ll << 20;

struct PendingSearch {
    bool active = false;
    const void* queries = nullptr;
    int q_dtype = 0;
    int64_t nq = 0;
    int k = 0;
    int64_t id_base = 0;
    float* out_scores = nullptr;
    int64_t* out_ids = nullptr;
    const int* q_label = nullptr;
    int n_qlab = 0;
    const int* q_map = nullptr;
    int slot = 0;
    size_t ev_begin = 0, ev_end = 0;
    int kx = 0;
    bool band = false;
    bool defer_flags = false;
    int lane = 0;
    float* l2_out = nullptr;
};

constexpr int FLAG_WORDS = 4;
constexpr int MAX_IN_FLIGHT = 4;
constexpr int64_t OVF_ROWS = 65536;

}

struct vodhip_index {
    int device = 0;
    int64_t dim = 0, dim_pad = 0;
    int64_t dim_s = 0;
    int64_t capacity = 0, capacity_pad = 0;
    int64_t ntotal = 0;
    int dtype = VODHIP_F16;
    uint16_t* data = nullptr;
    int* row_label = nullptr;
    const int* q_label = nullptr;
    int n_qlab = 0;
    void* stage_dev[2] = {nullptr, nullptr};
    void* stage_pin[2] = {nullptr, nullptr};
    hipEvent_t stage_done[2] = {nullptr, nullptr};
    int64_t ingest_threads = 0;
    int64_t last_ingest_pinned_src = 0;
    bool exact = false;
    float* data32 = nullptr;
    unsigned int* norm_stats = nullptr;
    float* row_n2 = nullptr;
    float* row_d2 = nullptr;
    bool stats_dirty = true;
    float ord_n2 = 0.f, ord_d2 = 0.f, cut_n2 = 0.f, cut_d2 = 0.f;
    int n_out = 0;
    int64_t exact_adapt = 1;
    int adapt_k = 0, adapt_kx = 0;
    int64_t last_exact_need = 0;
    float* x_list_s[4] = {nullptr, nullptr, nullptr, nullptr};
    int64_t* x_list_i[4] = {nullptr, nullptr, nullptr, nullptr};
    size_t x_list_cap[4] = {0, 0, 0, 0};
    float* x_eps = nullptr;
    unsigned int* x_flag_q = nullptr;
    int64_t exact_expand_x100 = 0;
    int64_t last_exact_kx = 0, last_exact_band_queries = 0, last_exact_band_passes = 0;
    bool l2 = false;
    unsigned int* l2_sat = nullptr;
    uint16_t* l2_q[4] = {nullptr, nullptr, nullptr, nullptr};
    float* l2_qn[4] = {nullptr, nullptr, nullptr, nullptr};
    float* l2_sim[4] = {nullptr, nullptr, nullptr, nullptr};
    size_t l2_q_cap[4] = {0, 0, 0, 0}, l2_qn_cap[4] = {0, 0, 0, 0}, l2_sim_cap[4] = {0, 0, 0, 0};
    hipEvent_t l2_ev[4][4] = {};
    int64_t last_l2_stage_ns = 0, last_l2_finish_ns = 0;
    SearchWorkspace ws_lane[2];
    hipStream_t lane_stream = nullptr;
    hipEvent_t lane_in[4] = {};
    int64_t lanes = 0;
    unsigned int* overflow_host = nullptr;
    unsigned int* ovf_q = nullptr;
    int* q_map = nullptr;
    hipEvent_t done[MAX_IN_FLIGHT] = {};
    std::deque<PendingSearch> inflight;
    int unfinished = 0;
    int next_slot = 0;
    PlanTunables tune;
    int64_t force_safe = 0;
    int64_t kflags = 0;
    int64_t profile = 0;
    int64_t last_overflow = 0, last_chunks = 0, last_survivor_ring = 0, last_ring_fallbacks = 0, last_safe_reruns = 0, last_recovered_queries = 0;
    int64_t last_filter_launches = 0, last_filter_ns = 0;
    int64_t last_recovery_launches = 0, last_recovery_ns = 0;
    std::atomic<int64_t> last_sample[6] = {};
    std::atomic<int64_t> last_sample_ns[5] = {};
    void* sample_ws = nullptr;
    size_t sample_ws_bytes = 0;
    std::mutex sample_mu;
    std::vector<hipEvent_t> ev_pool;
    size_t ev_used = 0;
    std::mutex mu;
};

namespace {

int elem_size(int dtype) { return dtype == VODHIP_F32 ? 4 : 2; }

int free_workspace(vodhip_index* ix, int lane) {
    SearchWorkspace& w = ix->ws_lane[lane];
    (void)hipFree(w.q_pad);
    (void)hipFree(w.topk);
    (void)hipFree(w.cand);
    (void)hipFree(w.cnt);
    (void)hipFree(w.thr_s);
    (void)hipFree(w.thr_key);
    (void)hipFree(w.overflow);
    (void)hipFree(w.ring);
    const int n_cu = w.n_cu;
    w = SearchWorkspace();
    w.n_cu = n_cu;
    return 0;
}

int ensure_workspace(vodhip_index* ix, int lane, int64_t nq_pad, int64_t cap, int64_t kp) {
    SearchWorkspace& w = ix->ws_lane[lane];
    if (w.nq_cap >= nq_pad && w.cap == cap && w.kp_cap >= kp && w.q_pad) {
        w.kp = kp;
        return 0;
    }
    const int64_t nq_cap = std::max(nq_pad, w.nq_cap);
    const int64_t kp_cap = std::max(kp, w.kp_cap);
    free_workspace(ix, lane);
    HIP_OK(hipMalloc((void**)&w.q_pad, (size_t)nq_cap * ix->dim_pad * 2));
    HIP_OK(hipMalloc((void**)&w.topk, (size_t)nq_cap * kp_cap * sizeof(key_t64)));
    HIP_OK(hipMalloc((void**)&w.cand, (size_t)nq_cap * cap * sizeof(key_t64)));
    HIP_OK(hipMalloc((void**)&w.cnt, (size_t)nq_cap * CNT_STRIDE * sizeof(unsigned int)));
    HIP_OK(hipMalloc((void**)&w.thr_s, (size_t)nq_cap * sizeof(float)));
    HIP_OK(hipMalloc((void**)&w.thr_key, (size_t)nq_cap * sizeof(key_t64)));
    HIP_OK(hipMalloc((void**)&w.overflow, FLAG_WORDS * sizeof(unsigned int)));
    w.nq_cap = nq_cap;
    w.cap = cap;
    w.kp = kp;
    w.kp_cap = kp_cap;
    return 0;
}

int ensure_ring(vodhip_index* ix, int lane, int64_t records) {
    SearchWorkspace& w = ix->ws_lane[lane];
    const int64_t floats = (int64_t)std::max(w.n_cu, 64) * 8 * records * 33;
    if (floats > w.ring_floats) {
        (void)hipFree(w.ring);
        w.ring = nullptr;
        w.ring_floats = 0;
        if (hipMalloc((void**)&w.ring, (size_t)floats * sizeof(float)) != hipSuccess) {
            (void)hipGetLastError();
            w.ring = nullptr;
            w.ring_cap = 0;
            return 0;
        }
        w.ring_floats = floats;
    }
    w.ring_cap = records;
    return 0;
}

void exact_bound_args(const vodhip_index* ix, ExactArgs& xa) {
    xa.ord_n2 = ix->ord_n2;
    xa.ord_d2 = ix->ord_d2;
    xa.cut_n2 = ix->cut_n2;
    xa.cut_d2 = ix->cut_d2;
    xa.n_out = ix->n_out;
    xa.out_rows = ix->norm_stats + EXS_OUT_ROWS;
    xa.row_n2 = ix->row_n2;
    xa.row_d2 = ix->row_d2;
}

int refresh_exact_stats(vodhip_index* ix, hipStream_t stream) {
    if (!ix->exact || !ix->stats_dirty) return 0;
    HIP_OK(launch_exact_stats(ix->row_n2, ix->row_d2, ix->ntotal, ix->norm_stats, stream));
    unsigned int w[8];
    HIP_OK(hipMemcpyAsync(w, ix->norm_stats, sizeof(w), hipMemcpyDeviceToHost, stream));
    HIP_OK(hipStreamSynchronize(stream));
    auto f = [](unsigned int u) { float v; memcpy(&v, &u, 4); return v; };
    ix->ord_n2 = f(w[EXS_ORD_N2]);
    ix->ord_d2 = f(w[EXS_ORD_D2]);
    ix->cut_n2 = f(w[EXS_CUT_N2]);
    ix->cut_d2 = f(w[EXS_CUT_D2]);
    ix->n_out = (int)std::min<unsigned int>(w[EXS_N_OUT], 2u * EXACT_MAX_OUTLIERS);
    if (w[EXS_N_OUT] > 2u * EXACT_MAX_OUTLIERS) return fail("internal error: %u outlier rows", w[EXS_N_OUT]);
    ix->stats_dirty = false;
    return 0;
}

int launch_stage(vodhip_index* ix, SearchWorkspace& W, const SearchPlan& plan, const Stage& sg, int64_t nq, int64_t nq_pad,
                 FilterStageFn experiment, hipStream_t stream) {
    hipEvent_t ev1 = nullptr;
    if (ix->profile) {
        while (ix->ev_pool.size() < ix->ev_used + 2) {
            hipEvent_t ev;
            HIP_OK(hipEventCreate(&ev));
            ix->ev_pool.push_back(ev);
        }
        hipEvent_t ev0 = ix->ev_pool[ix->ev_used++];
        ev1 = ix->ev_pool[ix->ev_used++];
        HIP_OK(hipEventRecord(ev0, stream));
    }
    W.extra.sample_rstride = (int)sg.rstride;
    W.extra.sample_offset = (int)sg.sample_offset;
    W.extra.sample_groups = (int)sg.n_groups;
    HIP_OK(launch_filter(ix->dtype, plan.kernel(sg, nq_pad), sg.kind, ix->data, W.q_pad, ix->dim_pad, sg.b, sg.e, sg.n_tiles, nq, nq_pad, W,
                         stream, experiment));
    if (ix->profile) HIP_OK(hipEventRecord(ev1, stream));
    return 0;
}

ExactArgs exact_stage_args(const vodhip_index* ix, const PendingSearch& ps, const SearchWorkspace& ws, int64_t row0, const Stage& sg, bool first) {
    ExactArgs xa;
    xa.plane = ix->data32;
    xa.stride = ix->dim_pad;
    xa.dim = (int)ix->dim;
    xa.dim_pad = (int)ix->dim_pad;
    xa.q_src = (const char*)ps.queries + (size_t)row0 * ix->dim * elem_size(ps.q_dtype);
    xa.q_dtype = ps.q_dtype;
    xa.q_map = ws.extra.q_map;
    xa.store_dtype = ix->dtype;
    exact_bound_args(ix, xa);
    xa.row_label = ws.extra.row_label;
    xa.q_label = ws.extra.q_label;
    xa.n_qlab = ws.extra.n_qlab;
    xa.mode = EXACT_CAND | (first ? EXACT_FIRST : 0);
    xa.cand = ws.cand;
    xa.cnt = ws.cnt;
    xa.cap = (int)ws.cap;
    xa.dense_n = sg.kind == ST_DENSE ? (int)(sg.e - sg.b) : -1;
    xa.thr_s = ws.thr_s;
    xa.thr_key = ws.thr_key;
    xa.kr = 2;
    while (xa.kr < ps.k) xa.kr <<= 1;
    xa.P = std::max(2 * xa.kr, 1024);
    xa.k = ps.k;
    xa.id_base = ps.id_base;
    xa.out_scores = ps.out_scores + row0 * ps.k;
    xa.out_ids = ps.out_ids + row0 * ps.k;
    xa.flag_word = ws.overflow;
    return xa;
}

int enqueue_search_impl(vodhip_index* ix, const PendingSearch& ps, bool safe, int recovery, hipStream_t stream) {
    SearchWorkspace& W = ix->ws_lane[ps.lane];
    const int k = ps.k;
    int64_t kp = 64;
    while (kp < k) kp <<= 1;
    const int64_t cap = ix->tune.cand_cap;
    if (cap / ROW_ALIGN * ROW_ALIGN < k) return fail("cand_cap=%lld is too small for k=%d", (long long)cap, k);

    const int* row_label = (ix->row_label && ps.q_label) ? ix->row_label : nullptr;
    PlanTunables tune = ix->tune;
    const FilterStageFn experiment = experiment_filter(tune);
    const SearchPlan plan = plan_search(ix->ntotal, k, ps.nq, tune, row_label != nullptr, safe, recovery);
    ix->last_chunks = (int64_t)plan.stages.size();
    ix->last_survivor_ring = plan.ring;

    const int q_es = elem_size(ps.q_dtype);
    if (ensure_workspace(ix, ps.lane, round_up(std::min(MAX_NQ_PER_PASS, ps.nq), 256), cap, kp)) return -1;
    if (ensure_ring(ix, ps.lane, plan.ring)) return -1;
    W.extra.flags = ((int)ix->kflags << 8) | (plan.corpus_nt ? FILTER_FLAG_CORPUS_NT : 0);
    W.extra.row_label = row_label;
    W.extra.n_qlab = ps.n_qlab;
    W.extra.perm_mul = (int)plan.perm_mul;
    W.extra.perm_mod = (int)plan.perm_mod;
    W.extra.row_bound = (int)ix->ntotal;
    const bool track_ovf = ps.nq <= OVF_ROWS;
    const SearchWorkspace& ws = W;
    for (int64_t qb = 0; qb < ps.nq; qb += MAX_NQ_PER_PASS) {
        const int64_t nq = std::min(MAX_NQ_PER_PASS, ps.nq - qb);
        const int64_t nq_pad = round_up(nq, plan.bn);
        const int* q_map = ps.q_map ? ps.q_map + qb : nullptr;
        const int64_t row0 = ps.q_map ? 0 : qb;
        W.ovf_q = track_ovf ? ix->ovf_q + (size_t)ps.slot * OVF_ROWS + qb : nullptr;
        const float* margin = ps.band ? ix->x_eps + (size_t)ps.slot * OVF_ROWS + row0 : nullptr;
        HIP_OK(launch_search_prepare(ws, (const char*)ps.queries + (size_t)row0 * ix->dim_s * q_es, ps.q_dtype, nq, ix->dim_s,
                                     ix->dtype, nq_pad, ix->dim_pad, qb == 0, recovery > 0 ? ps.out_scores + row0 * k : nullptr,
                                     recovery > 0 ? ps.out_ids + row0 * k : nullptr, k, q_map, stream, margin));
        W.extra.q_label = ps.q_label ? ps.q_label + (size_t)row0 * ps.n_qlab : nullptr;
        W.extra.q_map = q_map;
        for (size_t c = 0; c < plan.stages.size(); ++c) {
            const Stage& sg = plan.stages[c];
            if (launch_stage(ix, W, plan, sg, nq, nq_pad, experiment, stream)) return -1;
            if (ps.band) {
                HIP_OK(launch_exact_rescore(exact_stage_args(ix, ps, ws, row0, sg, c == 0), nq, stream));
                continue;
            }
            int64_t dense_n = -1;
            int flags = c + 1 == plan.stages.size() ? 1 : 0;
            if (sg.kind == ST_DENSE) dense_n = sg.e - sg.b;
            if (sg.kind == ST_GMAX) {
                dense_n = sg.n_groups;
                flags |= 2;
            }
            HIP_OK(launch_select(ws, nq, k, dense_n, flags, stream, ps.id_base, ps.out_scores + row0 * k, ps.out_ids + row0 * k, q_map));
        }
        if (plan.stages.empty())
            HIP_OK(launch_output(ws, nq, k, ps.id_base, ps.out_scores + qb * k, ps.out_ids + qb * k, stream));
    }
    if (ps.defer_flags) return 0;
    HIP_OK(hipMemcpyAsync(ix->overflow_host + FLAG_WORDS * ps.slot, ws.overflow, FLAG_WORDS * sizeof(unsigned int), hipMemcpyDeviceToHost, stream));
    HIP_OK(hipEventRecord(ix->done[ps.slot], stream));
    return 0;
}

int enqueue_search(vodhip_index* ix, const PendingSearch& ps, bool safe, int recovery, hipStream_t stream) {
    const int rc = enqueue_search_impl(ix, ps, safe, recovery, stream);
    if (rc) (void)hipStreamSynchronize(stream);
    return rc;
}

int exact_kx(const vodhip_index* ix, int k, bool upper_limit = false) {
    const int64_t x100 = ix->exact_expand_x100 > 0 ? ix->exact_expand_x100 : ((ix->dtype == VODHIP_F16 && !upper_limit) ? 110 : 200);
    const int64_t kx = ((int64_t)k * x100 + 99) / 100 + 16;
    const int64_t fits = std::max<int64_t>(k, ix->tune.cand_cap / ROW_ALIGN * ROW_ALIGN);
    return (int)std::min<int64_t>(std::min<int64_t>(VODHIP_MAX_K, fits), std::max<int64_t>(kx, k));
}

PendingSearch exact_inner(const vodhip_index* ix, const PendingSearch& ps) {
    PendingSearch in = ps;
    in.k = ps.kx;
    in.kx = 0;
    in.id_base = 0;
    in.out_scores = ix->x_list_s[ps.slot];
    in.out_ids = ix->x_list_i[ps.slot];
    in.defer_flags = false;
    return in;
}

int enqueue_exact_list(vodhip_index* ix, const PendingSearch& ps, hipStream_t stream) {
    ExactArgs xa;
    xa.plane = ix->data32;
    xa.stride = ix->dim_pad;
    xa.dim = (int)ix->dim;
    xa.dim_pad = (int)ix->dim_pad;
    xa.q_src = ps.queries;
    xa.q_dtype = ps.q_dtype;
    xa.store_dtype = ix->dtype;
    exact_bound_args(ix, xa);
    xa.row_label = (ix->row_label && ps.q_label) ? ix->row_label : nullptr;
    xa.q_label = ps.q_label;
    xa.n_qlab = ps.n_qlab;
    xa.mode = EXACT_LIST;
    xa.list_s = ix->x_list_s[ps.slot];
    xa.list_i = ix->x_list_i[ps.slot];
    xa.kx = ps.kx;
    xa.P = 64;
    while (xa.P < ps.kx + xa.n_out) xa.P <<= 1;
    xa.k = ps.k;
    xa.id_base = ps.id_base;
    xa.out_scores = ps.out_scores;
    xa.out_ids = ps.out_ids;
    xa.eps = ix->x_eps + (size_t)ps.slot * OVF_ROWS;
    xa.flag_word = ix->ws_lane[ps.lane].overflow + 1;
    xa.flag_q = ix->x_flag_q + (size_t)ps.slot * OVF_ROWS;
    HIP_OK(launch_exact_rescore(xa, ps.nq, stream));
    HIP_OK(hipMemcpyAsync(ix->overflow_host + FLAG_WORDS * ps.slot, ix->ws_lane[ps.lane].overflow, FLAG_WORDS * sizeof(unsigned int), hipMemcpyDeviceToHost, stream));
    HIP_OK(hipEventRecord(ix->done[ps.slot], stream));
    return 0;
}

int exact_reserve_lists(vodhip_index* ix, int slot, size_t elems) {
    if (ix->x_list_cap[slot] >= elems) return 0;
    (void)hipFree(ix->x_list_s[slot]);
    (void)hipFree(ix->x_list_i[slot]);
    ix->x_list_s[slot] = nullptr;
    ix->x_list_i[slot] = nullptr;
    ix->x_list_cap[slot] = 0;
    HIP_OK(hipMalloc((void**)&ix->x_list_s[slot], elems * sizeof(float)));
    HIP_OK(hipMalloc((void**)&ix->x_list_i[slot], elems * sizeof(int64_t)));
    ix->x_list_cap[slot] = elems;
    return 0;
}

template <typename T>
int l2_reserve(T*& buf, size_t& cap, size_t elems) {
    if (cap >= elems) return 0;
    (void)hipFree(buf);
    buf = nullptr;
    cap = 0;
    HIP_OK(hipMalloc((void**)&buf, elems * sizeof(T)));
    cap = elems;
    return 0;
}

int l2_profile_mark(vodhip_index* ix, int slot, int which, hipStream_t stream) {
    if (!ix->profile) return 0;
    if (!ix->l2_ev[slot][which]) HIP_OK(hipEventCreate(&ix->l2_ev[slot][which]));
    HIP_OK(hipEventRecord(ix->l2_ev[slot][which], stream));
    return 0;
}

int enqueue_l2_finish(vodhip_index* ix, const PendingSearch& ps, hipStream_t stream) {
    HIP_OK(launch_l2_finish(ix->l2_sim[ps.slot], ix->l2_qn[ps.slot], ps.nq, ps.k, ps.l2_out, stream));
    return 0;
}

}

extern "C" {

const char* vodhip_last_error(void) { return g_last_error.c_str(); }
int vodhip_version(void) { return VODHIP_VERSION; }

int vodhip_index_create(int device, int64_t dim, int store_dtype, int64_t capacity_rows, vodhip_index_t** out) {
    if (!out) return fail("out is NULL");
    if (dim <= 0 || capacity_rows < 0) return fail("invalid dim=%lld / capacity=%lld", (long long)dim, (long long)capacity_rows);
    const bool exact = (store_dtype & VODHIP_EXACT_F32) != 0;
    const bool l2 = (store_dtype & VODHIP_L2) != 0;
    store_dtype &= ~(VODHIP_EXACT_F32 | VODHIP_L2);
    if (store_dtype != VODHIP_F16 && store_dtype != VODHIP_BF16) return fail("store dtype must be F16 or BF16 (optionally | VODHIP_EXACT_F32 or | VODHIP_L2)");
    if (l2 && exact) return fail("VODHIP_L2 | VODHIP_EXACT_F32 is not supported: an L2 store scores the rounded rows (DESIGN.md 8)");
    if (exact && (dim + 63) / 64 * 64 > 16384) return fail("VODHIP_EXACT_F32 stores take dim <= 16384");
    if (capacity_rows >= (1ll << 31) - 2 * ROW_ALIGN) return fail("capacity must be < 2^31 rows per device");
    HIP_OK(hipSetDevice(device));
    vodhip_index* ix = new vodhip_index();
    ix->device = device;
    ix->dim = dim;
    ix->l2 = l2;
    ix->dim_s = l2 ? dim + L2_BIAS_COLS : dim;
    ix->dim_pad = round_up(ix->dim_s, 64);
    ix->capacity = capacity_rows;
    ix->capacity_pad = round_up(capacity_rows, ROW_ALIGN) + 2 * ROW_ALIGN;
    ix->dtype = store_dtype;
    ix->exact = exact;
    if (hipDeviceGetAttribute(&ix->tune.n_cu, hipDeviceAttributeMultiprocessorCount, device) != hipSuccess || ix->tune.n_cu < 1) ix->tune.n_cu = 256;
    ix->ws_lane[0].n_cu = ix->ws_lane[1].n_cu = ix->tune.n_cu;
    const size_t bytes = (size_t)ix->capacity_pad * ix->dim_pad * 2;
    hipError_t e = hipMalloc((void**)&ix->data, bytes);
    if (e != hipSuccess) {
        delete ix;
        return fail("hipMalloc of the %zu-byte vector store failed: %s", bytes, hipGetErrorString(e));
    }
    e = hipMemset(ix->data, 0, bytes);
    if (e == hipSuccess) e = hipStreamSynchronize(nullptr);
    if (e == hipSuccess) e = hipMalloc((void**)&ix->ovf_q, MAX_IN_FLIGHT * OVF_ROWS * sizeof(unsigned int));
    if (e == hipSuccess) e = hipMalloc((void**)&ix->q_map, MAX_IN_FLIGHT * OVF_ROWS * sizeof(int));
    if (e == hipSuccess) e = hipHostMalloc((void**)&ix->overflow_host, FLAG_WORDS * MAX_IN_FLIGHT * sizeof(unsigned int), hipHostMallocDefault);
    for (int i = 0; i < MAX_IN_FLIGHT && e == hipSuccess; ++i) e = hipEventCreateWithFlags(&ix->done[i], hipEventDisableTiming);
    for (int i = 0; i < MAX_IN_FLIGHT && e == hipSuccess; ++i) e = hipEventCreateWithFlags(&ix->lane_in[i], hipEventDisableTiming);
    if (e == hipSuccess) e = hipStreamCreateWithFlags(&ix->lane_stream, hipStreamNonBlocking);
    if (l2 && e == hipSuccess) e = hipMalloc((void**)&ix->l2_sat, sizeof(unsigned int));
    if (l2 && e == hipSuccess) e = hipMemset(ix->l2_sat, 0, sizeof(unsigned int));
    if (l2 && e == hipSuccess) e = hipStreamSynchronize(nullptr);
    if (exact && e == hipSuccess) {
        const size_t bytes32 = ((size_t)capacity_rows + 1) * ix->dim_pad * sizeof(float);
        e = hipMalloc((void**)&ix->data32, bytes32);
        if (e != hipSuccess) {
            (void)hipGetLastError();
            (void)hipFree(ix->data);
            (void)hipFree(ix->ovf_q);
            (void)hipFree(ix->q_map);
            (void)hipHostFree(ix->overflow_host);
            delete ix;
            return fail("hipMalloc of the %zu-byte float32 plane (VODHIP_EXACT_F32) failed: %s", bytes32, hipGetErrorString(e));
        }
        if (e == hipSuccess) e = hipMalloc((void**)&ix->norm_stats, EXS_WORDS * sizeof(unsigned int));
        if (e == hipSuccess) e = hipMemset(ix->norm_stats, 0, EXS_WORDS * sizeof(unsigned int));
        if (e == hipSuccess) e = hipMalloc((void**)&ix->row_n2, ((size_t)capacity_rows + 1) * sizeof(float));
        if (e == hipSuccess) e = hipMalloc((void**)&ix->row_d2, ((size_t)capacity_rows + 1) * sizeof(float));
        if (e == hipSuccess) e = hipMalloc((void**)&ix->x_eps, MAX_IN_FLIGHT * OVF_ROWS * sizeof(float));
        if (e == hipSuccess) e = hipMalloc((void**)&ix->x_flag_q, MAX_IN_FLIGHT * OVF_ROWS * sizeof(unsigned int));
        if (e == hipSuccess) e = hipStreamSynchronize(nullptr);
    }
    if (e != hipSuccess) {
        (void)hipGetLastError();
        (void)hipFree(ix->data);
        (void)hipFree(ix->data32);
        (void)hipFree(ix->l2_sat);
        delete ix;
        return fail("store initialisation failed: %s", hipGetErrorString(e));
    }
    for (int i = 0; i < FLAG_WORDS * MAX_IN_FLIGHT; ++i) ix->overflow_host[i] = 0;
    *out = ix;
    return 0;
}

int vodhip_index_destroy(vodhip_index_t* ix) {
    if (!ix) return 0;
    (void)hipSetDevice(ix->device);
    if (!ix->inflight.empty()) (void)hipDeviceSynchronize();
    free_workspace(ix, 0);
    free_workspace(ix, 1);
    if (ix->lane_stream) (void)hipStreamDestroy(ix->lane_stream);
    for (int i = 0; i < MAX_IN_FLIGHT; ++i)
        if (ix->lane_in[i]) (void)hipEventDestroy(ix->lane_in[i]);
    for (hipEvent_t e : ix->ev_pool) (void)hipEventDestroy(e);
    for (int i = 0; i < MAX_IN_FLIGHT; ++i)
        if (ix->done[i]) (void)hipEventDestroy(ix->done[i]);
    (void)hipFree(ix->data);
    for (int b = 0; b < 2; ++b) {
        (void)hipFree(ix->stage_dev[b]);
        (void)hipHostFree(ix->stage_pin[b]);
        if (ix->stage_done[b]) (void)hipEventDestroy(ix->stage_done[b]);
    }
    (void)hipFree(ix->data32);
    (void)hipFree(ix->norm_stats);
    (void)hipFree(ix->row_n2);
    (void)hipFree(ix->row_d2);
    (void)hipFree(ix->x_eps);
    (void)hipFree(ix->x_flag_q);
    for (int i = 0; i < MAX_IN_FLIGHT; ++i) {
        (void)hipFree(ix->x_list_s[i]);
        (void)hipFree(ix->x_list_i[i]);
    }
    (void)hipFree(ix->l2_sat);
    for (int i = 0; i < MAX_IN_FLIGHT; ++i)
        for (hipEvent_t e : ix->l2_ev[i])
            if (e) (void)hipEventDestroy(e);
    for (int i = 0; i < MAX_IN_FLIGHT; ++i) {
        (void)hipFree(ix->l2_q[i]);
        (void)hipFree(ix->l2_qn[i]);
        (void)hipFree(ix->l2_sim[i]);
    }
    (void)hipFree(ix->row_label);
    (void)hipFree(ix->sample_ws);
    (void)hipFree(ix->ovf_q);
    (void)hipFree(ix->q_map);
    (void)hipHostFree(ix->overflow_host);
    delete ix;
    return 0;
}

int vodhip_index_add(vodhip_index_t* ix, const void* rows, int64_t n_rows, int src_dtype, int src_location, void* stream_) {
    if (!ix) return fail("index is NULL");
    if (n_rows < 0 || (n_rows > 0 && !rows)) return fail("invalid rows");
// ... 183 lines not shown
    return 0;
}

int vodhip_index_search_async(vodhip_index_t* ix, const void* queries, int q_dtype, int64_t nq, int k, int64_t id_base,
                              float* out_scores, int64_t* out_ids, void* stream_) {
    if (!ix) return fail("index is NULL");
    if (k < 1 || k > VODHIP_MAX_K) return fail("k=%d out of range [1, %d]", k, VODHIP_MAX_K);
    if (nq < 0 || (nq > 0 && (!queries || !out_scores || !out_ids))) return fail("invalid query / output pointers");
    if (q_dtype < 0 || q_dtype > 2) return fail("invalid q_dtype %d", q_dtype);
    std::lock_guard<std::mutex> guard(ix->mu);
    if (ix->tune.cand_cap < ROW_ALIGN || ix->tune.cand_cap < k) return fail("cand_cap too small");
    if ((int)ix->inflight.size() + ix->unfinished >= MAX_IN_FLIGHT)
        return fail("%d searches are already in flight on this index: call vodhip_index_search_finish first", MAX_IN_FLIGHT);
    if (ix->exact && nq > OVF_ROWS) return fail("VODHIP_EXACT_F32: at most %lld queries per search", (long long)OVF_ROWS);
    HIP_OK(hipSetDevice(ix->device));
    PendingSearch ps;
    ps.active = true;
    ps.queries = queries;
    ps.q_dtype = q_dtype;
    ps.nq = nq;
    ps.k = k;
    ps.id_base = id_base;
    ps.out_scores = out_scores;
    ps.out_ids = out_ids;
    ps.q_label = ix->q_label;
    ps.n_qlab = ix->n_qlab;
    ps.slot = ix->next_slot;
    hipStream_t stream = (hipStream_t)stream_;
    if (ix->exact && nq > 0 && refresh_exact_stats(ix, stream)) return -1;
    const int64_t lanes_eff = ix->lanes > 0 ? ix->lanes : (nq <= 256 ? 2 : 1);
    if (lanes_eff == 2 && nq > 0) {
        ps.lane = ix->inflight.empty() ? 0 : 1 - ix->inflight.back().lane;
        if (ps.lane == 1) {
            HIP_OK(hipEventRecord(ix->lane_in[ps.slot], stream));
            HIP_OK(hipStreamWaitEvent(ix->lane_stream, ix->lane_in[ps.slot], 0));
            stream = ix->lane_stream;
        }
    }
    if (ix->inflight.empty() && ix->unfinished == 0) ix->ev_used = 0;
    ps.ev_begin = ix->ev_used;
    if (ix->l2 && nq > 0) {
        if (l2_reserve(ix->l2_q[ps.slot], ix->l2_q_cap[ps.slot], (size_t)nq * ix->dim_s)) return -1;
        if (l2_reserve(ix->l2_qn[ps.slot], ix->l2_qn_cap[ps.slot], (size_t)nq)) return -1;
        if (l2_reserve(ix->l2_sim[ps.slot], ix->l2_sim_cap[ps.slot], (size_t)nq * k)) return -1;
        if (l2_profile_mark(ix, ps.slot, 0, stream)) return -1;
        HIP_OK(launch_l2_stage_queries(queries, q_dtype, nq, ix->dim, ix->dtype, ix->l2_q[ps.slot], ix->l2_qn[ps.slot], stream));
        if (l2_profile_mark(ix, ps.slot, 1, stream)) return -1;
        ps.queries = ix->l2_q[ps.slot];
        ps.q_dtype = ix->dtype;
        ps.l2_out = out_scores;
        ps.out_scores = ix->l2_sim[ps.slot];
        PendingSearch first = ps;
        first.defer_flags = true;
        if (enqueue_search(ix, first, ix->force_safe != 0, 0, stream)) return -1;
        const SearchWorkspace& ws = ix->ws_lane[ps.lane];
        if (l2_profile_mark(ix, ps.slot, 2, stream) || enqueue_l2_finish(ix, ps, stream) || l2_profile_mark(ix, ps.slot, 3, stream) ||
            hipMemcpyAsync(ix->overflow_host + FLAG_WORDS * ps.slot, ws.overflow, FLAG_WORDS * sizeof(unsigned int), hipMemcpyDeviceToHost, stream) != hipSuccess ||
            hipEventRecord(ix->done[ps.slot], stream) != hipSuccess) {
            (void)hipGetLastError();
            (void)hipStreamSynchronize(stream);
            return fail("enqueueing the L2 finish failed");
        }
    } else if (ix->exact && nq > 0) {
        const int kx_formula = exact_kx(ix, k);
        const bool adapt = ix->exact_adapt && ix->exact_expand_x100 == 0 && ix->adapt_k == k && ix->adapt_kx >= k;
        const int kx_limit = exact_kx(ix, k, true);
        ps.kx = adapt ? std::min(ix->adapt_kx, kx_limit) : kx_formula;
        if (exact_reserve_lists(ix, ps.slot, (size_t)nq * kx_limit)) return -1;
        PendingSearch in = exact_inner(ix, ps);
        in.defer_flags = true;
        if (enqueue_search(ix, in, ix->force_safe != 0, 0, stream)) return -1;
        if (enqueue_exact_list(ix, ps, stream)) {
            (void)hipStreamSynchronize(stream);
            return -1;
        }
    } else if (nq > 0 && enqueue_search(ix, ps, ix->force_safe != 0, 0, stream)) {
        return -1;
    }
    ps.ev_end = ix->ev_used;
    ix->next_slot = (ix->next_slot + 1) % MAX_IN_FLIGHT;
    ix->inflight.push_back(ps);
    return 0;
}

namespace {

int recover_overflow(vodhip_index* ix, const PendingSearch& ps, hipStream_t stream) {
    PendingSearch rs = ps;
    int pass = 0;
    while (ix->overflow_host[FLAG_WORDS * ps.slot]) {
        if (++pass > 40) return fail("internal error: the exhaustive schedule overflowed");
        ix->last_overflow = 1;
        ix->last_safe_reruns += 1;
        if (pass == 1 && ps.nq <= OVF_ROWS && !ps.band) {
            std::vector<unsigned int> flags((size_t)ps.nq);
            HIP_OK(hipMemcpy(flags.data(), ix->ovf_q + (size_t)ps.slot * OVF_ROWS, (size_t)ps.nq * sizeof(unsigned int), hipMemcpyDeviceToHost));
            std::vector<int> rows;
            for (int64_t q = 0; q < ps.nq; ++q)
                if (flags[(size_t)q]) rows.push_back((int)q);
            ix->last_recovered_queries = rows.empty() ? ps.nq : (int64_t)rows.size();
            if (!rows.empty() && (int64_t)rows.size() < ps.nq) {
                int* dmap = ix->q_map + (size_t)ps.slot * OVF_ROWS;
                HIP_OK(hipMemcpy(dmap, rows.data(), rows.size() * sizeof(int), hipMemcpyHostToDevice));
                rs.q_map = dmap;
                rs.nq = (int64_t)rows.size();
            }
        }
        const size_t ev_first = ix->ev_used;
        if (enqueue_search(ix, rs, false, pass + (ps.band ? 1 : 0), stream)) return -1;
        HIP_OK(hipStreamSynchronize(stream));
        for (size_t e = ev_first; e + 1 < ix->ev_used; e += 2) {
            float ms = 0.f;
            HIP_OK(hipEventElapsedTime(&ms, ix->ev_pool[e], ix->ev_pool[e + 1]));
            ix->last_recovery_ns += (int64_t)((double)ms * 1e6);
            ++ix->last_recovery_launches;
        }
        ix->ev_used = ev_first;
    }
    return pass;
}

}

int vodhip_index_search_finish(vodhip_index_t* ix, void* stream_) {
    if (!ix) return fail("index is NULL");
    hipStream_t stream = (hipStream_t)stream_;
    std::unique_lock<std::mutex> guard(ix->mu);
    if (ix->inflight.empty()) return fail("no search is pending on this index");
    HIP_OK(hipSetDevice(ix->device));
    PendingSearch ps = ix->inflight.front();
    ix->inflight.pop_front();
    if (ps.lane == 1) stream = ix->lane_stream;
    if (ps.nq > 0) {
        ++ix->unfinished;
        guard.unlock();
        const hipError_t ev_rc = hipEventSynchronize(ix->done[ps.slot]);
        guard.lock();
        --ix->unfinished;
        HIP_OK(ev_rc);
    }
    ix->last_overflow = 0;
    ix->last_safe_reruns = 0;
    ix->last_recovered_queries = 0;
    ix->last_recovery_launches = 0;
    ix->last_recovery_ns = 0;
    ix->last_exact_kx = ps.kx;
    ix->last_exact_band_queries = 0;
    ix->last_exact_band_passes = 0;
    ix->last_exact_need = ps.kx > 0 && ps.nq > 0 ? (int64_t)ix->overflow_host[FLAG_WORDS * ps.slot + 2] : 0;
    ix->last_ring_fallbacks = ps.nq > 0 ? (int64_t)ix->overflow_host[FLAG_WORDS * ps.slot + 3] : 0;
    if (ps.kx > 0 && ps.nq > 0 && ix->exact_adapt && ix->exact_expand_x100 == 0) {
        const int need = (int)ix->overflow_host[FLAG_WORDS * ps.slot + 2];
        const int formula = exact_kx(ix, ps.k), limit = exact_kx(ix, ps.k, true);
        int target = need >= ps.kx ? std::min(limit, (ps.kx + ps.kx / 4 + 7) / 8 * 8) : std::min(limit, (need + need / 16 + 8 + 7) / 8 * 8);
        target = std::max(target, std::min(formula, ps.k + 8));
        if (ix->adapt_k != ps.k || ix->adapt_kx <= 0) ix->adapt_kx = formula;
        ix->adapt_k = ps.k;
        ix->adapt_kx = target >= ix->adapt_kx ? target : ix->adapt_kx - std::max(8, (ix->adapt_kx - target) / 4 / 8 * 8);
        if (ix->adapt_kx < target) ix->adapt_kx = target;
    }
    if (ps.nq > 0 && ps.kx == 0) {
        const int passes = recover_overflow(ix, ps, stream);
        if (passes < 0) return -1;
        if (passes > 0 && ps.l2_out) {
            if (enqueue_l2_finish(ix, ps, stream)) return -1;
            HIP_OK(hipStreamSynchronize(stream));
        }
    } else if (ps.nq > 0) {
        const int passes = recover_overflow(ix, exact_inner(ix, ps), stream);
        if (passes < 0) return -1;
        if (passes > 0) {
            if (enqueue_exact_list(ix, ps, stream)) return -1;
            HIP_OK(hipStreamSynchronize(stream));
        }
        if (ix->overflow_host[FLAG_WORDS * ps.slot + 1]) {
            std::vector<unsigned int> flags((size_t)ps.nq);
            HIP_OK(hipMemcpy(flags.data(), ix->x_flag_q + (size_t)ps.slot * OVF_ROWS, (size_t)ps.nq * sizeof(unsigned int), hipMemcpyDeviceToHost));
            std::vector<int> rows;
            for (int64_t q = 0; q < ps.nq; ++q)
                if (flags[(size_t)q]) rows.push_back((int)q);
            ix->last_exact_band_queries = (int64_t)rows.size();
            if (!rows.empty()) {
                PendingSearch bs = ps;
                bs.band = true;
                bs.kx = 0;
                int* dmap = ix->q_map + (size_t)ps.slot * OVF_ROWS;
                if ((int64_t)rows.size() < ps.nq) {
                    HIP_OK(hipMemcpy(dmap, rows.data(), rows.size() * sizeof(int), hipMemcpyHostToDevice));
                    bs.q_map = dmap;
                    bs.nq = (int64_t)rows.size();
                }
                const size_t ev_first = ix->ev_used;
                if (enqueue_search(ix, bs, false, 1, stream)) return -1;
                HIP_OK(hipStreamSynchronize(stream));
                for (size_t e = ev_first; e + 1 < ix->ev_used; e += 2) {
                    float ms = 0.f;
                    HIP_OK(hipEventElapsedTime(&ms, ix->ev_pool[e], ix->ev_pool[e + 1]));
                    ix->last_recovery_ns += (int64_t)((double)ms * 1e6);
                    ++ix->last_recovery_launches;
                }
                ix->ev_used = ev_first;
                const int more = recover_overflow(ix, bs, stream);
                if (more < 0) return -1;
                ix->last_exact_band_passes = 1 + more;
            }
        }
    }
    ix->last_l2_stage_ns = ix->last_l2_finish_ns = 0;
    if (ps.l2_out && ps.nq > 0 && ix->profile && ix->l2_ev[ps.slot][0] && ix->l2_ev[ps.slot][3]) {
        float ms = 0.f;
        HIP_OK(hipEventElapsedTime(&ms, ix->l2_ev[ps.slot][0], ix->l2_ev[ps.slot][1]));
        ix->last_l2_stage_ns = (int64_t)((double)ms * 1e6);
        HIP_OK(hipEventElapsedTime(&ms, ix->l2_ev[ps.slot][2], ix->l2_ev[ps.slot][3]));
        ix->last_l2_finish_ns = (int64_t)((double)ms * 1e6);
    }
    ix->last_filter_launches = (int64_t)((ps.ev_end - ps.ev_begin) / 2);
    ix->last_filter_ns = 0;
    for (size_t e = ps.ev_begin; e + 1 < ps.ev_end; e += 2) {
        float ms = 0.f;
        HIP_OK(hipEventElapsedTime(&ms, ix->ev_pool[e], ix->ev_pool[e + 1]));
        ix->last_filter_ns += (int64_t)((double)ms * 1e6);
    }
    return 0;
}

int vodhip_index_search(vodhip_index_t* ix, const void* queries, int q_dtype, int64_t nq, int k, int64_t id_base,
                        float* out_scores, int64_t* out_ids, void* stream) {
    if (vodhip_index_search_async(ix, queries, q_dtype, nq, k, id_base, out_scores, out_ids, stream)) return -1;
    return vodhip_index_search_finish(ix, stream);
}

static int listed_check(vodhip_index_t* ix, const void* queries, int q_dtype, int64_t nq, const int64_t* ids_dev, int64_t m,
                        const int32_t* q_labels_dev, int n_per_query) {
    if (!ix) return fail("index is NULL");
    if (ix->l2) return fail("listed ids are not supported on an L2 index (VODHIP_L2): score_ids / search_ids need an inner-product store");
    if (m < 1) return fail("m=%lld: a list holds at least one slot", (long long)m);
    if (nq < 0 || (nq > 0 && (!queries || !ids_dev))) return fail("invalid query / id pointers");
    if (q_dtype < 0 || q_dtype > 2) return fail("invalid q_dtype %d", q_dtype);
    if (q_labels_dev && (n_per_query < 1 || n_per_query > 64)) return fail("n_per_query must be in [1, 64]");
    if (q_labels_dev && !ix->row_label) return fail("set the row labels first (vodhip_index_set_row_labels)");
    return 0;
}

static int listed_score(vodhip_index_t* ix, const void* queries, int q_dtype, int64_t nq, const int64_t* ids_dev, int64_t m,
                        int64_t id_base, const int32_t* q_labels_dev, int n_per_query, float* out, hipStream_t stream) {
    ListedArgs a;
    a.plane = ix->exact ? (const void*)ix->data32 : (const void*)ix->data;
    a.stride = ix->dim_pad;
    a.dim = (int)ix->dim;
    a.dim_pad = (int)ix->dim_pad;
    a.store_dtype = ix->dtype;
    a.exact = ix->exact ? 1 : 0;
    a.q_src = queries;
    a.q_dtype = q_dtype;
    a.ids = ids_dev;
    a.m = m;
    a.id_base = id_base;
    a.ntotal = ix->ntotal;
    a.row_label = ix->row_label;
    a.q_label = q_labels_dev;
    a.n_qlab = q_labels_dev ? n_per_query : 0;
    a.out = out;
    HIP_OK(launch_score_listed(a, nq, stream));
    return 0;
}

int vodhip_index_score_ids(vodhip_index_t* ix, const void* queries, int q_dtype, int64_t nq, const int64_t* ids_dev, int64_t m,
                           int64_t id_base, const int32_t* q_labels_dev, int n_per_query, float* out_scores, void* stream_) {
    if (listed_check(ix, queries, q_dtype, nq, ids_dev, m, q_labels_dev, n_per_query)) return -1;
    if (nq > 0 && !out_scores) return fail("out_scores is NULL");
    if (nq == 0) return 0;
    HIP_OK(hipSetDevice(ix->device));
    return listed_score(ix, queries, q_dtype, nq, ids_dev, m, id_base, q_labels_dev, n_per_query, out_scores, (hipStream_t)stream_);
}
// ... 352 lines not shown
            for (int i = 0; i < 5 && le == hipSuccess; ++i) {
                float ms = 0.f;
                le = hipEventElapsedTime(&ms, ev[i], ev[i + 1]);
                ns[i] += (double)ms * 1e6;
            }
        }
    }
    unsigned int st[8] = {};
    if (le == hipSuccess) le = hipMemcpyAsync(st, a.status, sizeof(st), hipMemcpyDeviceToHost, stream);
    if (le != hipSuccess) (void)hipGetLastError();
    const hipError_t se = hipStreamSynchronize(stream);
    for (int i = 0; i < 6; ++i)
        if (ev[i]) (void)hipEventDestroy(ev[i]);
    if (le != hipSuccess) return fail("sample-posterior launch failed: %s", hipGetErrorString(le));
    HIP_OK(se);
    ix->last_sample[0] = st[0];
    ix->last_sample[1] = st[1];
    ix->last_sample[2] = st[2];
    ix->last_sample[3] = st[3];
    ix->last_sample[4] = (int64_t)(((uint64_t)st[5] << 32) | st[4]);
    ix->last_sample[5] = emit_groups;
    for (int i = 0; i < 5; ++i) ix->last_sample_ns[i] = (int64_t)ns[i];
    if (st[0]) return fail("candidate list overflow: %u queries met more than %d tile maxima tied with their threshold", st[0], VODHIP_SAMPLE_SLACK_TILES);
    return 0;
}

int vodhip_debug_schedule(int64_t ntotal, int k, int64_t nq, int64_t cand_cap, int64_t dense_rows, int64_t sample_div,
                          int64_t growth_x100, int tile, int recovery_pass, int n_cu, int64_t* out, int max_stages) {
    PlanTunables t;
    if (cand_cap > 0) t.cand_cap = cand_cap;
    if (dense_rows > 0) t.dense_rows = round_up(dense_rows, ROW_ALIGN);
    if (sample_div > 0) t.sample_div = sample_div;
    t.growth_x100 = growth_x100;
    t.tile = tile;
    if (n_cu > 0) t.n_cu = n_cu;
    if (!out || max_stages < 1 || k < 1 || nq < 1 || ntotal < 0 || (tile != 0 && !find_kernel(tile) && !experiment_filter(t)))
        return fail("invalid arguments");
    const std::vector<Stage> st = plan_search(ntotal, k, nq, t, false, false, recovery_pass).stages;
    if ((int)st.size() > max_stages) return fail("%d stages do not fit max_stages=%d", (int)st.size(), max_stages);
    for (size_t i = 0; i < st.size(); ++i) {
        const int64_t row[6] = {st[i].kind, st[i].b, st[i].e, st[i].n_tiles, st[i].rstride, st[i].n_groups};
        memcpy(out + i * 6, row, sizeof(row));
    }
    return (int)st.size();
}

int vodhip_debug_tile_order(int64_t ntotal, int64_t* perm_mul, int64_t* perm_mod) {
    if (!perm_mul || !perm_mod || ntotal < 0) return fail("invalid arguments");
    *perm_mod = (ntotal + ROW_ALIGN - 1) / ROW_ALIGN;
    *perm_mul = tile_order_multiplier(*perm_mod);
    return 0;
}

int vodhip_index_set_param(vodhip_index_t* ix, const char* key, int64_t value) {
    if (!ix || !key) return fail("NULL argument");
    if (!strcmp(key, "cand_cap")) {
        if (value < ROW_ALIGN || value > (1 << 16)) return fail("cand_cap must be in [256, 65536]");
        ix->tune.cand_cap = value;
    } else if (!strcmp(key, "dense_rows")) {
        if (value < ROW_ALIGN) return fail("dense_rows must be >= 256");
        ix->tune.dense_rows = round_up(value, ROW_ALIGN);
    } else if (!strcmp(key, "growth")) {
        ix->tune.growth_x100 = value;
    } else if (!strcmp(key, "force_safe")) {
        ix->force_safe = value;
    } else if (!strcmp(key, "small_chunk_tiles")) {
        ix->tune.small_chunk_tiles = value;
    } else if (!strcmp(key, "kflags")) {
        ix->kflags = value;
    } else if (!strcmp(key, "sample_div")) {
        if (value != 0 && value < 2) return fail("sample_div must be 0 (auto) or >= 2");
        ix->tune.sample_div = value;
    } else if (!strcmp(key, "profile")) {
        ix->profile = value;
    } else if (!strcmp(key, "ingest_threads")) {
        if (value < 0 || value > 256) return fail("ingest_threads must be in [0, 256] (0 = auto)");
        ix->ingest_threads = value;
    } else if (!strcmp(key, "lanes")) {
        if (value < 0 || value > 2) return fail("lanes must be 0 (auto: 2 for batches of one query tile), 1 or 2");
        if (!ix->inflight.empty()) return fail("searches are in flight: finish them before changing the lanes");
        ix->lanes = value;
    } else if (!strcmp(key, "survivor_ring")) {
        if (value < 0 || value > MAX_SURVIVOR_RING) return fail("survivor_ring must be in [0, 8192] (0 = auto)");
        ix->tune.survivor_ring = value;
    } else if (!strcmp(key, "tile_order")) {
        if (value != 0 && value != 1) return fail("tile_order must be 0 (low-discrepancy stage order) or 1 (row order)");
        ix->tune.tile_order = value;
    } else if (!strcmp(key, "exact_adapt")) {
        if (value < 0 || value > 1) return fail("exact_adapt must be 0 or 1");
        ix->exact_adapt = value;
        ix->adapt_k = ix->adapt_kx = 0;
    } else if (!strcmp(key, "exact_expand")) {
        if (value < 0 || value > 100000) return fail("exact_expand (x100) must be in [0, 100000]");
        ix->exact_expand_x100 = value;
    } else if (!strcmp(key, "tile")) {
        PlanTunables t;
        t.tile = value;
        if (value != 0 && !find_kernel(value) && !experiment_filter(t))
            return fail("tile must be 0 (auto) or a filter-kernel variant id: 1, 8, 9, 14, 42, 46 (DESIGN.md 4)");
        ix->tune.tile = value;
    } else {
        return fail("unknown parameter '%s'", key);
    }
    return 0;
}

int vodhip_index_get_stat(const vodhip_index_t* ix, const char* key, int64_t* out) {
    if (!ix || !key || !out) return fail("NULL argument");
    if (!strcmp(key, "last_overflow"))
        *out = ix->last_overflow;
    else if (!strcmp(key, "last_chunks"))
        *out = ix->last_chunks;
    else if (!strcmp(key, "last_survivor_ring"))
        *out = ix->last_survivor_ring;
    else if (!strcmp(key, "last_ring_fallbacks"))
        *out = ix->last_ring_fallbacks;
    else if (!strcmp(key, "last_safe_reruns"))
        *out = ix->last_safe_reruns;
    else if (!strcmp(key, "last_recovered_queries"))
        *out = ix->last_recovered_queries;
    else if (!strcmp(key, "last_filter_launches"))
        *out = ix->last_filter_launches;
    else if (!strcmp(key, "last_filter_ns"))
        *out = ix->last_filter_ns;
    else if (!strcmp(key, "last_recovery_launches"))
        *out = ix->last_recovery_launches;
    else if (!strcmp(key, "last_recovery_ns"))
        *out = ix->last_recovery_ns;
    else if (!strcmp(key, "last_sample_overflow"))
        *out = ix->last_sample[0];
    else if (!strcmp(key, "last_sample_selfcheck"))
        *out = ix->last_sample[1];
    else if (!strcmp(key, "last_sample_max_candidates"))
        *out = ix->last_sample[2];
    else if (!strcmp(key, "last_sample_emit_skipped"))
        *out = ix->last_sample[3];
    else if (!strcmp(key, "last_sample_candidates"))
        *out = ix->last_sample[4];
    else if (!strcmp(key, "last_sample_emit_groups"))
        *out = ix->last_sample[5];
    else if (!strcmp(key, "last_sample_ns_partition"))
        *out = ix->last_sample_ns[0];
    else if (!strcmp(key, "last_sample_ns_keymax"))
        *out = ix->last_sample_ns[1];
    else if (!strcmp(key, "last_sample_ns_threshold"))
        *out = ix->last_sample_ns[2];
    else if (!strcmp(key, "last_sample_ns_emit"))
        *out = ix->last_sample_ns[3];
    else if (!strcmp(key, "last_sample_ns_select"))
        *out = ix->last_sample_ns[4];
    else if (!strcmp(key, "exact"))
        *out = ix->exact ? 1 : 0;
    else if (!strcmp(key, "l2"))
        *out = ix->l2 ? 1 : 0;
    else if (!strcmp(key, "last_l2_stage_ns"))
        *out = ix->last_l2_stage_ns;
    else if (!strcmp(key, "last_l2_finish_ns"))
        *out = ix->last_l2_finish_ns;
    else if (!strcmp(key, "l2_saturated_rows")) {
        unsigned int w = 0;
        if (ix->l2) {
            HIP_OK(hipSetDevice(ix->device));
            HIP_OK(hipDeviceSynchronize());
            HIP_OK(hipMemcpy(&w, ix->l2_sat, sizeof(w), hipMemcpyDeviceToHost));
        }
        *out = (int64_t)w;
    } else if (!strcmp(key, "last_exact_kx"))
        *out = ix->last_exact_kx;
    else if (!strcmp(key, "last_exact_need"))
        *out = ix->last_exact_need;
    else if (!strcmp(key, "exact_outliers")) {
        *out = ix->n_out;
    } else if (!strcmp(key, "last_exact_band_queries"))
        *out = ix->last_exact_band_queries;
    else if (!strcmp(key, "last_exact_band_passes"))
        *out = ix->last_exact_band_passes;
    else if (!strcmp(key, "cand_cap"))
        *out = ix->tune.cand_cap;
// ... 618 lines not shown
```

### vod_amd/csrc/vodhip_internal.h

```cpp
#pragma once
#include <hip/hip_runtime.h>
#include <stdint.h>

#include "search_plan.h"

#ifdef VODHIP_ABLATION
#define VODHIP_PROBE(buf, i)                                                  \
    do {                                                                      \
        if (blockIdx.x == 0 && threadIdx.x == 0) {                            \
            (buf)[2 * (i)] = (long long)__builtin_amdgcn_s_memtime();         \
            (buf)[2 * (i) + 1] = (long long)__builtin_amdgcn_s_memrealtime(); \
        }                                                                     \
    } while (0)
#define VODHIP_PROBE_WG(buf, end)                                                                                   \
    do {                                                                                                            \
        if (blockIdx.x < 64 && threadIdx.x == 0) (buf)[128 + 2 * blockIdx.x + (end)] = (long long)__builtin_amdgcn_s_memrealtime(); \
    } while (0)
#else
#define VODHIP_PROBE_WG(buf, end) \
    do {                          \
    } while (0)
#define VODHIP_PROBE(buf, i) \
    do {                     \
    } while (0)
#endif

namespace vodhip {

void set_last_error(const char* msg);

hipError_t read_probe_hybrid(long long* out);
hipError_t read_probe_sample(int which, long long* out);
hipError_t read_probe_select(long long* out);

typedef unsigned long long key_t64;

constexpr int CNT_STRIDE = 32;

enum : int { FILTER_FLAG_CORPUS_NT = 1 };

struct FilterExtra {
    int flags = 0;
    const int* row_label = nullptr;
    const int* q_label = nullptr;
    int n_qlab = 0;
    int sample_rstride = 0;
    int sample_offset = 0;
    int sample_groups = 0;
    const int* q_map = nullptr;
    int perm_mul = 0, perm_mod = 0, row_bound = 0;
};

struct SearchWorkspace {
    uint16_t* q_pad = nullptr;
    key_t64* topk = nullptr;
    key_t64* cand = nullptr;
    unsigned int* cnt = nullptr;
    float* thr_s = nullptr;
    key_t64* thr_key = nullptr;
    unsigned int* overflow = nullptr;
    unsigned int* ovf_q = nullptr;
    float* ring = nullptr;
    int64_t ring_floats = 0;
    int64_t ring_cap = 0;
    int n_cu = 256;
    int64_t nq_cap = 0;
    int64_t cap = 0;
    int64_t kp = 0;
    int64_t kp_cap = 0;
    FilterExtra extra;
};

hipError_t launch_convert_rows(const void* src, int src_dtype, int64_t n_rows, int64_t dim, void* dst, int dst_dtype,
                               int64_t dst_stride, hipStream_t stream);
hipError_t launch_search_prepare(const SearchWorkspace& ws, const void* q_src, int q_dtype, int64_t nq, int64_t dim,
                                 int store_dtype, int64_t nq_pad, int64_t dim_pad, bool clear_overflow,
                                 const float* seed_scores, const int64_t* seed_ids, int k, const int* q_map, hipStream_t stream,
                                 const float* seed_margin = nullptr);
hipError_t launch_select(const SearchWorkspace& ws, int64_t nq, int k, int64_t dense_n, int flags, hipStream_t stream,
                         int64_t id_base = 0, float* out_scores = nullptr, int64_t* out_ids = nullptr, const int* q_map = nullptr);
hipError_t launch_output(const SearchWorkspace& ws, int64_t nq, int k, int64_t id_base, float* out_scores,
                         int64_t* out_ids, hipStream_t stream);
hipError_t launch_merge_topk(const float* scores, const int64_t* ids, int64_t stride_s, int64_t stride_i, int n_shards,
                             int64_t nq, int k, int k_out, float* out_scores, int64_t* out_ids, hipStream_t stream);
hipError_t allow_dynamic_lds(const void* kernel, int bytes);
hipError_t launch_filter_8phase(int store_dtype, int lead, bool keep_b0, const void* store, const void* q_pad, int64_t dim_pad, int64_t row_begin,
                                int64_t row_end, int64_t nq, int64_t nq_pad, const SearchWorkspace& ws, hipStream_t stream);
using FilterStageFn = hipError_t (*)(int store_dtype, const void* store, const void* q_pad, int64_t dim_pad, int64_t row_begin, int64_t row_end,
                                     int64_t nq, int64_t nq_pad, const SearchWorkspace& ws, hipStream_t stream);
#ifdef VODHIP_EXPERIMENTS
FilterStageFn experiment_filter(PlanTunables& t);
#else
inline FilterStageFn experiment_filter(PlanTunables&) { return nullptr; }
#endif
hipError_t launch_filter(int store_dtype, FilterKernel kernel, int mode, const void* store, const void* q_pad, int64_t dim_pad,
                         int64_t row_begin, int64_t row_end, int64_t n_sample_tiles, int64_t nq, int64_t nq_pad,
                         const SearchWorkspace& ws, hipStream_t stream, FilterStageFn experiment = nullptr);

enum : int { EXACT_LIST = 0, EXACT_CAND = 1, EXACT_FIRST = 2 };
struct ExactArgs {
    const float* plane = nullptr;
    int64_t stride = 0;
    int dim = 0, dim_pad = 0;
    const void* q_src = nullptr;
    int q_dtype = 0;
    const int* q_map = nullptr;
    int store_dtype = 0;
    float ord_n2 = 0.f, ord_d2 = 0.f;
    float cut_n2 = 0.f, cut_d2 = 0.f;
    int n_out = 0;
    const unsigned int* out_rows = nullptr;
    const float* row_n2 = nullptr;
    const float* row_d2 = nullptr;
    const int* row_label = nullptr;
    const int* q_label = nullptr;
    int n_qlab = 0;
    int mode = EXACT_LIST;
    const float* list_s = nullptr;
    const int64_t* list_i = nullptr;
    int kx = 0;
    const key_t64* cand = nullptr;
    unsigned int* cnt = nullptr;
    int cap = 0, dense_n = -1;
    float* thr_s = nullptr;
    key_t64* thr_key = nullptr;
    int kr = 0;
    int P = 0;
    int k = 0;
    int64_t id_base = 0;
    float* out_scores = nullptr;
    int64_t* out_ids = nullptr;
    float* eps = nullptr;
    unsigned int* flag_word = nullptr;
    unsigned int* flag_q = nullptr;
};
constexpr int EXACT_MAX_OUTLIERS = 32;
enum : int { EXS_MAX_N2 = 0, EXS_MAX_D2 = 1, EXS_ORD_N2 = 2, EXS_ORD_D2 = 3, EXS_N_OUT = 4, EXS_CUT_N2 = 5, EXS_CUT_D2 = 6,
             EXS_HIST_N2 = 8, EXS_HIST_D2 = 24, EXS_OUT_ROWS = 64, EXS_WORDS = 64 + 2 * EXACT_MAX_OUTLIERS };
hipError_t launch_ingest_exact(const void* src, int src_dtype, int64_t n_rows, int64_t dim, void* dst16, int dst_dtype, float* dst32,
                               int64_t stride, unsigned int* stats, float* row_n2, float* row_d2, hipStream_t stream);
hipError_t launch_exact_stats(const float* row_n2, const float* row_d2, int64_t n_rows, unsigned int* stats, hipStream_t stream);
hipError_t launch_exact_rescore(const ExactArgs& a, int64_t nq, hipStream_t stream);

struct ListedArgs {
    const void* plane = nullptr;
    int64_t stride = 0;
    int dim = 0, dim_pad = 0;
    int store_dtype = 0;
    int exact = 0;
    const void* q_src = nullptr;
    int q_dtype = 0;
    const int64_t* ids = nullptr;
    int64_t m = 0, id_base = 0, ntotal = 0;
    const int* row_label = nullptr;
    const int* q_label = nullptr;
    int n_qlab = 0;
    float* out = nullptr;
    int spb = 0;
    int64_t chunks = 0;
    const float* weights = nullptr;
    float* part = nullptr;
};
hipError_t launch_score_listed(ListedArgs a, int64_t nq, hipStream_t stream);
int64_t listed_sum_chunks(int64_t m);
hipError_t launch_sum_listed(ListedArgs a, int64_t nq, hipStream_t stream);
hipError_t launch_fold_listed_sum(const float* parts, int64_t n_parts, int64_t part_stride, int64_t q_stride, int64_t nq, int dim, float* out,
                                  hipStream_t stream);
hipError_t launch_combine_listed(const float* parts, const int64_t* ids, int64_t n, int n_shards, int64_t rows_per_shard, float* out,
                                 hipStream_t stream);
hipError_t launch_select_listed(const float* scores, const int64_t* ids, int64_t nq, int64_t m, int k, int64_t id_base, float* out_scores,
                                int64_t* out_ids, hipStream_t stream);

hipError_t launch_l2_bias(void* rows, int store_dtype, int64_t n_rows, int64_t dim, int64_t stride, unsigned int* saturated,
                          hipStream_t stream);
hipError_t launch_l2_stage_queries(const void* q_src, int q_dtype, int64_t nq, int64_t dim, int store_dtype, void* staged, float* qn,
                                   hipStream_t stream);
hipError_t launch_l2_finish(const float* sim, const float* qn, int64_t nq, int k, float* dist, hipStream_t stream);

struct ScanInputs {
    const void* store = nullptr;
    int64_t dim = 0, dim_pad = 0, ntotal = 0;
    int store_dtype = 0;
    const void* q_src = nullptr;
    int q_dtype = 0;
    const int* row_label = nullptr;
    const int* q_label = nullptr;
    int n_qlab = 0;
    void* q_stage = nullptr;
};
int64_t scan_nq_pad(int64_t nq);
int64_t scan_tiles(int64_t ntotal);
hipError_t launch_scan_stage(const ScanInputs& s, int64_t q_first, int64_t nq, int64_t nq_pad, hipStream_t stream);
FilterExtra scan_filter_extra(const ScanInputs& s, int64_t q_first);

struct PartitionArgs : ScanInputs {
    float beta = 1.f;
    void* part = nullptr;
    float* out_max = nullptr;
    float* out_log_rel = nullptr;
};
hipError_t launch_log_partition(const PartitionArgs& a, int64_t q_first, int64_t nq, hipStream_t stream);

struct RankArgs : ScanInputs {
    int64_t m = 0, id_base = 0;
    const int64_t* ids = nullptr;
    const float* thresholds = nullptr;
    const int64_t* tie_ids = nullptr;
    void* mini = nullptr;
    int* slot_row = nullptr;
    unsigned int* table = nullptr;
    float* out_score = nullptr;
    int* out_rows = nullptr;
    int64_t* out_count = nullptr;
};
enum : int { RANK_MODE_PICK = 0, RANK_MODE_RANK = 1, RANK_MODE_THRESHOLDS = 2 };
int64_t rank_mini_rows(int64_t nq_pad, int64_t m);
hipError_t launch_rank(const RankArgs& a, int mode, int64_t q_first, int64_t nq, hipStream_t stream);

struct PosteriorArgs {
    PartitionArgs p;
    float* acc = nullptr;
    float* out_mean = nullptr;
};
int64_t posterior_mean_groups(int64_t ntotal);
hipError_t launch_posterior_mean(const PosteriorArgs& a, int64_t q_first, int64_t nq, hipStream_t stream);

struct PosteriorSampleArgs {
    PartitionArgs p;
    int k = 0;
    uint64_t seed = 0;
// ... 142 lines not shown
```

Baseline: 81200 queries/s.

## Publish status flags from kernels to host memory and add in-kernel wall-clock stamps

The final select, exact-rescore and L2-finish kernels now write the overflow/status words directly into a device-visible host buffer, using a last-block ticket or block 0. This removes the separate device-to-host memcpy of the flag words after each search. Profiling also gains in-kernel wall-clock stamps recorded per filter launch as an alternative to HIP events. The cost is extra atomics and a slightly larger workspace, plus added complexity around when the host can trust the published status.

```diff
diff --git a/include/vodhip.h b/include/vodhip.h
--- a/include/vodhip.h
+++ b/include/vodhip.h
@@ -92,6 +92,7 @@
 int vodhip_debug_schedule(int64_t ntotal, int k, int64_t nq, int64_t cand_cap, int64_t dense_rows, int64_t sample_div,
                           int64_t growth_x100, int tile, int recovery_pass, int n_cu, int64_t* out, int max_stages);
 int vodhip_index_get_stat(const vodhip_index_t* index, const char* key, int64_t* out);
+int vodhip_debug_stamp_ns(uint64_t start_ticks, uint64_t end_ticks, int64_t rate_khz, int64_t* ns);
 int vodhip_debug_l2_split(float c, int dtype, uint16_t terms[3], float consts[3]);
 int vodhip_debug_tile_order(int64_t ntotal, int64_t* perm_mul, int64_t* perm_mod);
 int vodhip_debug_read_probe(int which, int64_t* out, int n);
diff --git a/vod_amd/_native.py b/vod_amd/_native.py
--- a/vod_amd/_native.py
+++ b/vod_amd/_native.py
@@ -72,6 +72,7 @@
     "vodhip_index_set_param": (_i32, [_vp, _c.c_char_p, _i64]),
     "vodhip_debug_schedule": (_i32, [_i64, _i32, _i64, _i64, _i64, _i64, _i64, _i32, _i32, _i32, _c.POINTER(_i64), _i32]),
     "vodhip_index_get_stat": (_i32, [_vp, _c.c_char_p, _c.POINTER(_i64)]),
+    "vodhip_debug_stamp_ns": (_i32, [_c.c_uint64, _c.c_uint64, _i64, _c.POINTER(_i64)]),
     "vodhip_debug_l2_split": (_i32, [_c.c_float, _i32, _c.POINTER(_c.c_uint16), _c.POINTER(_c.c_float)]),
     "vodhip_debug_tile_order": (_i32, [_i64, _c.POINTER(_i64), _c.POINTER(_i64)]),
     "vodhip_debug_read_probe": (_i32, [_i32, _c.POINTER(_i64), _i32]),
diff --git a/vod_amd/csrc/kernels_exact.hip b/vod_amd/csrc/kernels_exact.hip
--- a/vod_amd/csrc/kernels_exact.hip
+++ b/vod_amd/csrc/kernels_exact.hip
@@ -375,6 +375,7 @@
             if ((unsigned)need_s > __hip_atomic_load(a.flag_word + 1, __ATOMIC_RELAXED, __HIP_MEMORY_SCOPE_AGENT)) atomicMax(a.flag_word + 1, (unsigned)need_s);
         }
     }
+    if (!cand_mode) publish_status(a.status, a.status_out);
 }
 
 hipError_t launch_exact_rescore(const ExactArgs& a, int64_t nq, hipStream_t stream) {
diff --git a/vod_amd/csrc/kernels_l2.hip b/vod_amd/csrc/kernels_l2.hip
--- a/vod_amd/csrc/kernels_l2.hip
+++ b/vod_amd/csrc/kernels_l2.hip
@@ -86,8 +86,10 @@
     }
 }
 
-__global__ void __launch_bounds__(256) l2_finish_kernel(const float* __restrict__ sim, const float* __restrict__ qn, int64_t nq, int k, float* __restrict__ dist) {
+__global__ void __launch_bounds__(256) l2_finish_kernel(const float* __restrict__ sim, const float* __restrict__ qn, int64_t nq, int k, float* __restrict__ dist,
+                                                        const unsigned int* __restrict__ status, StatusOut status_out) {
     const int64_t i = (int64_t)blockIdx.x * blockDim.x + threadIdx.x;
+    publish_settled_status(status, status_out);
     if (i >= nq * k) return;
     const float s = sim[i];
     float d = __builtin_inff();
@@ -121,10 +123,11 @@
     return hipGetLastError();
 }
 
-hipError_t launch_l2_finish(const float* sim, const float* qn, int64_t nq, int k, float* dist, hipStream_t stream) {
+hipError_t launch_l2_finish(const float* sim, const float* qn, int64_t nq, int k, float* dist, hipStream_t stream, const unsigned int* status,
+                            StatusOut status_out) {
     if (nq == 0) return hipSuccess;
     const int64_t n = nq * k;
-    hipLaunchKernelGGL(l2_finish_kernel, dim3((unsigned)((n + 255) / 256)), dim3(256), 0, stream, sim, qn, nq, k, dist);
+    hipLaunchKernelGGL(l2_finish_kernel, dim3((unsigned)((n + 255) / 256)), dim3(256), 0, stream, sim, qn, nq, k, dist, status, status_out);
     return hipGetLastError();
 }
 
diff --git a/vod_amd/csrc/kernels_mips.hip b/vod_amd/csrc/kernels_mips.hip
--- a/vod_amd/csrc/kernels_mips.hip
+++ b/vod_amd/csrc/kernels_mips.hip
@@ -40,6 +40,7 @@
     const int qt = jj % n_qtiles;
     const int xt = (jj / n_qtiles) * 8 + xcd;
     if (xt >= n_xtiles) return;
+    filter_stamp_begin(ex, overflow);
 
     const int tid = threadIdx.x;
     const int lane = tid & 63;
@@ -201,6 +202,7 @@
             }
         }
     }
+    filter_stamp_end(ex, overflow);
 }
 
 constexpr int WSTG_CAP = 256;
@@ -226,6 +228,7 @@
     const int xt0 = (jj / n_qtiles) * 8 + xcd;
     const int xt_step = (int)gridDim.x / n_qtiles;
     if (xt0 >= n_xtiles) return;
+    filter_stamp_begin(ex, overflow);
     const int n_my = (n_xtiles - 1 - xt0) / xt_step + 1;
     const int tid = threadIdx.x;
     const int lane = tid & 63;
@@ -480,6 +483,7 @@
         }
     }
     if constexpr (MODE == MODE_FILTER) wl.flush(out);
+    filter_stamp_end(ex, overflow);
 }
 
 __device__ __forceinline__ void bitonic_sort_desc_lds(key_t64* keys, int P, int tid) {
@@ -649,7 +653,7 @@
                                                           float* __restrict__ thr_s, key_t64* __restrict__ thr_key,
                                                           unsigned int* __restrict__ overflow, unsigned int* __restrict__ ovf_q, int flags,
                                                           int64_t id_base, float* __restrict__ out_scores,
-                                                          int64_t* __restrict__ out_ids, const int* __restrict__ q_map) {
+                                                          int64_t* __restrict__ out_ids, const int* __restrict__ q_map, StatusOut status_out) {
     extern __shared__ __attribute__((aligned(16))) char smem[];
     int* hist = (int*)smem;
     key_t64* front = (key_t64*)(hist + SEL_HIST_INTS);
@@ -672,6 +676,7 @@
         if (tid == 0) {
             atomicOr(overflow, 1u);
             if (ovf_q) ovf_q[q] = 1u;
+            if (status_out.host) status_out.host[0] = 1u;
         }
         n = cap;
     }
@@ -754,6 +759,7 @@
         g_probe_select[2 * (pb + 6) + 1] = 1;
 #endif
     }
+    publish_settled_status(overflow, status_out);
 }
 
 __global__ void mips_output_kernel(const key_t64* __restrict__ topk, int kp, int k, int64_t nq, int64_t id_base,
@@ -868,7 +874,13 @@
         thr_s[i] = ts;
         thr_key[i] = tk;
     }
+    if (i < FILTER_STAMP_SLOTS && clear_overflow) {
+        unsigned long long* const pair = (unsigned long long*)(overflow + FILTER_FLAG_WORDS) + 2 * i;
+        pair[0] = ~0ull;
+        pair[1] = 0ull;
+    }
     if (i == 0 && clear_overflow) {
+        overflow[FILTER_TICKET_WORD] = 0u;
         overflow[0] = 0u;
         overflow[1] = 0u;
         overflow[2] = 0u;
@@ -1005,24 +1017,24 @@
 
 template <int KPT>
 static hipError_t launch_select_kpt(const SearchWorkspace& ws, int64_t nq, int k, int64_t dense_n, int flags, hipStream_t stream,
-                                    int64_t id_base, float* out_scores, int64_t* out_ids, const int* q_map) {
+                                    int64_t id_base, float* out_scores, int64_t* out_ids, const int* q_map, StatusOut status_out) {
     const size_t lds = SEL_HIST_INTS * sizeof(int) + (size_t)ws.kp * sizeof(key_t64);
     const bool final_sort = (flags & SELECT_FINAL) != 0;
     hipLaunchKernelGGL(mips_select_kernel<KPT>, dim3((unsigned)nq), dim3(256), lds, stream, ws.topk, (int)ws.kp, k, ws.cand,
                        ws.cnt, (int)ws.cap, (int)dense_n, ws.thr_s, ws.thr_key, ws.overflow, ws.ovf_q, flags, id_base,
-                       final_sort ? out_scores : nullptr, final_sort ? out_ids : nullptr, q_map);
+                       final_sort ? out_scores : nullptr, final_sort ? out_ids : nullptr, q_map, status_out);
     return hipGetLastError();
 }
 
 hipError_t launch_select(const SearchWorkspace& ws, int64_t nq, int k, int64_t dense_n, int flags, hipStream_t stream,
-                         int64_t id_base, float* out_scores, int64_t* out_ids, const int* q_map) {
+                         int64_t id_base, float* out_scores, int64_t* out_ids, const int* q_map, StatusOut status_out) {
     int sb = 2048;
     while (sb < 2 * ws.kp) sb <<= 1;
     while (dense_n > sb - ws.kp && sb < 8192) sb <<= 1;
     switch (sb) {
-        case 2048: return launch_select_kpt<8>(ws, nq, k, dense_n, flags, stream, id_base, out_scores, out_ids, q_map);
-        case 4096: return launch_select_kpt<16>(ws, nq, k, dense_n, flags, stream, id_base, out_scores, out_ids, q_map);
-        default: return launch_select_kpt<32>(ws, nq, k, dense_n, flags, stream, id_base, out_scores, out_ids, q_map);
+        case 2048: return launch_select_kpt<8>(ws, nq, k, dense_n, flags, stream, id_base, out_scores, out_ids, q_map, status_out);
+        case 4096: return launch_select_kpt<16>(ws, nq, k, dense_n, flags, stream, id_base, out_scores, out_ids, q_map, status_out);
+        default: return launch_select_kpt<32>(ws, nq, k, dense_n, flags, stream, id_base, out_scores, out_ids, q_map, status_out);
     }
 }
 
diff --git a/vod_amd/csrc/kernels_mips_8phase.hip b/vod_amd/csrc/kernels_mips_8phase.hip
--- a/vod_amd/csrc/kernels_mips_8phase.hip
+++ b/vod_amd/csrc/kernels_mips_8phase.hip
@@ -33,6 +33,7 @@
     const int xt0 = (jj / n_qtiles) * 8 + xcd;
     const int xt_step = (int)gridDim.x / n_qtiles;
     if (xt0 >= n_xtiles) return;
+    const unsigned long long stamp_t0 = filter_stamp_now(ex);
     const int n_my = (n_xtiles - 1 - xt0) / xt_step + 1;
     const int tid = threadIdx.x;
     const int lane = tid & 63;
@@ -129,6 +130,7 @@
 #pragma unroll
     for (int j = 0; j < NB16; ++j) asm volatile("" : "+v"(thr[j]));
     wait_vmcnt<0>();
+    filter_stamp<false>(ex, overflow, stamp_t0);
 
     WaveSurvivorList<P8_WL_CAP, SUBSET> wl(smem + P8_OPERANDS, NWAVES, wave);
     const SurvivorOut out{thr_key, cand, cnt, cap, overflow, ex};
@@ -433,6 +435,7 @@
 #endif
     wl_flush();
     if (ring_fallbacks > 0 && lane == 0) atomicAdd(overflow + 3, (unsigned)ring_fallbacks);
+    filter_stamp_end(ex, overflow);
 }
 
 template <bool KEEPB0, int LEAD = 7>
diff --git a/vod_amd/csrc/mips_common.h b/vod_amd/csrc/mips_common.h
--- a/vod_amd/csrc/mips_common.h
+++ b/vod_amd/csrc/mips_common.h
@@ -97,6 +97,47 @@
     const unsigned long long pos = (unsigned long long)(row_begin / 256 + xt / per);
     const int super = (int)((pos * (unsigned long long)ex.perm_mul) % (unsigned long long)ex.perm_mod);
     return super * 256 + (xt % per) * BM;
+}
+
+__device__ __forceinline__ unsigned long long filter_stamp_now(const FilterExtra& ex) {
+    return ex.stamp_slot < 0 ? 0ull : (unsigned long long)wall_clock64();
+}
+template <bool END>
+__device__ __forceinline__ void filter_stamp(const FilterExtra& ex, unsigned int* flag_words, unsigned long long now) {
+    if (ex.stamp_slot < 0) return;
+    if constexpr (END) __syncthreads();
+    if (threadIdx.x == 0) {
+        unsigned long long* const pair = (unsigned long long*)(flag_words + FILTER_FLAG_WORDS) + 2 * ex.stamp_slot;
+        if constexpr (END) atomicMax(pair + 1, (unsigned long long)wall_clock64());
+        else atomicMin(pair, now);
+    }
+}
+__device__ __forceinline__ void filter_stamp_begin(const FilterExtra& ex, unsigned int* flag_words) {
+    filter_stamp<false>(ex, flag_words, filter_stamp_now(ex));
+}
+__device__ __forceinline__ void filter_stamp_end(const FilterExtra& ex, unsigned int* flag_words) { filter_stamp<true>(ex, flag_words, 0ull); }
+
+__device__ __forceinline__ void publish_status(unsigned int* status, const StatusOut& so) {
+    if (so.host == nullptr) return;
+    __shared__ unsigned int publish_last;
+    if (threadIdx.x == 0) {
+        wait_vmcnt<0>();
+        publish_last = atomicAdd(status + FILTER_TICKET_WORD, 1u) + 1u == gridDim.x ? 1u : 0u;
+    }
+    __syncthreads();
+    if (publish_last) {
+        for (int w = (int)threadIdx.x; w < so.n_words; w += (int)blockDim.x)
+            so.host[w] = __hip_atomic_load(status + w, __ATOMIC_RELAXED, __HIP_MEMORY_SCOPE_AGENT);
+        if (threadIdx.x == 0) status[FILTER_TICKET_WORD] = 0u;
+    }
+}
+
+__device__ __forceinline__ void publish_settled_status(const unsigned int* status, const StatusOut& so) {
+    if (so.host == nullptr || blockIdx.x != 0) return;
+    for (int w = (int)threadIdx.x; w < so.n_words; w += (int)blockDim.x) {
+        const unsigned v = __hip_atomic_load(status + w, __ATOMIC_RELAXED, __HIP_MEMORY_SCOPE_AGENT);
+        if (w != 0 || v != 0u) so.host[w] = v;
+    }
 }
 
 __device__ __forceinline__ bool subset_allows(const FilterExtra& ex, int q, int row) {
diff --git a/vod_amd/csrc/vodhip_api.hip b/vod_amd/csrc/vodhip_api.hip
--- a/vod_amd/csrc/vodhip_api.hip
+++ b/vod_amd/csrc/vodhip_api.hip
@@ -75,9 +75,13 @@
     bool defer_flags = false;
     int lane = 0;
     float* l2_out = nullptr;
+    int n_stamps = 0;
+    int n_stages = 0;
 };
 
-constexpr int FLAG_WORDS = 4;
+constexpr int FLAG_WORDS = FILTER_FLAG_WORDS;
+constexpr int STAGE_STATS = 64;
+constexpr int SLOT_WORDS = FILTER_STATUS_WORDS;
 constexpr int MAX_IN_FLIGHT = 4;
 constexpr int64_t OVF_ROWS = 65536;
 
@@ -129,6 +133,7 @@
     hipStream_t lane_stream = nullptr;
     hipEvent_t lane_in[4] = {};
     int64_t lanes = 0;
+    unsigned int* overflow_host_dev = nullptr;
     unsigned int* overflow_host = nullptr;
     unsigned int* ovf_q = nullptr;
     int* q_map = nullptr;
@@ -140,6 +145,10 @@
     int64_t force_safe = 0;
     int64_t kflags = 0;
     int64_t profile = 0;
+    int64_t profile_events = 0;
+    int64_t wall_khz = 0;
+    int enq_stamps = 0, enq_stages = 0;
+    int64_t last_stage_ns[STAGE_STATS] = {};
     int64_t last_overflow = 0, last_chunks = 0, last_survivor_ring = 0, last_ring_fallbacks = 0, last_safe_reruns = 0, last_recovered_queries = 0;
     int64_t last_filter_launches = 0, last_filter_ns = 0;
     int64_t last_recovery_launches = 0, last_recovery_ns = 0;
@@ -188,7 +197,7 @@
     HIP_OK(hipMalloc((void**)&w.cnt, (size_t)nq_cap * CNT_STRIDE * sizeof(unsigned int)));
     HIP_OK(hipMalloc((void**)&w.thr_s, (size_t)nq_cap * sizeof(float)));
     HIP_OK(hipMalloc((void**)&w.thr_key, (size_t)nq_cap * sizeof(key_t64)));
-    HIP_OK(hipMalloc((void**)&w.overflow, FLAG_WORDS * sizeof(unsigned int)));
+    HIP_OK(hipMalloc((void**)&w.overflow, FILTER_WORKSPACE_WORDS * sizeof(unsigned int)));
     w.nq_cap = nq_cap;
     w.cap = cap;
     w.kp = kp;
@@ -244,9 +253,11 @@
 }
 
 int launch_stage(vodhip_index* ix, SearchWorkspace& W, const SearchPlan& plan, const Stage& sg, int64_t nq, int64_t nq_pad,
-                 FilterStageFn experiment, hipStream_t stream) {
+                 FilterStageFn experiment, hipStream_t stream, int stamp_slot) {
     hipEvent_t ev1 = nullptr;
-    if (ix->profile) {
+    const bool events = ix->profile && stamp_slot < 0;
+    W.extra.stamp_slot = stamp_slot;
+    if (events) {
         while (ix->ev_pool.size() < ix->ev_used + 2) {
             hipEvent_t ev;
             HIP_OK(hipEventCreate(&ev));
@@ -261,8 +272,33 @@
     W.extra.sample_groups = (int)sg.n_groups;
     HIP_OK(launch_filter(ix->dtype, plan.kernel(sg, nq_pad), sg.kind, ix->data, W.q_pad, ix->dim_pad, sg.b, sg.e, sg.n_tiles, nq, nq_pad, W,
                          stream, experiment));
-    if (ix->profile) HIP_OK(hipEventRecord(ev1, stream));
-    return 0;
+    if (events) HIP_OK(hipEventRecord(ev1, stream));
+    return 0;
+}
+
+StatusOut status_out(const vodhip_index* ix, int slot, int n_stamps) {
+    StatusOut so;
+    if (ix->overflow_host_dev) {
+        so.host = ix->overflow_host_dev + SLOT_WORDS * slot;
+        so.n_words = FLAG_WORDS + 4 * n_stamps;
+    }
+    return so;
+}
+
+int enqueue_status_copy(vodhip_index* ix, int slot, int lane, int n_stamps, hipStream_t stream) {
+    HIP_OK(hipMemcpyAsync(ix->overflow_host + SLOT_WORDS * slot, ix->ws_lane[lane].overflow, (size_t)(FLAG_WORDS + 4 * n_stamps) * sizeof(unsigned int),
+                          hipMemcpyDeviceToHost, stream));
+    return 0;
+}
+
+void read_stamps(const vodhip_index* ix, int slot, int n, int n_stages, int64_t* total, int64_t* by_stage) {
+    uint64_t pair[2];
+    for (int l = 0; l < n; ++l) {
+        memcpy(pair, ix->overflow_host + SLOT_WORDS * slot + FLAG_WORDS + 4 * l, sizeof(pair));
+        const int64_t ns = std::max<int64_t>(0, filter_stamp_ns(pair[0], pair[1], ix->wall_khz));
+        *total += ns;
+        if (by_stage && n_stages > 0) by_stage[std::min(l % n_stages, STAGE_STATS - 1)] += ns;
+    }
 }
 
 ExactArgs exact_stage_args(const vodhip_index* ix, const PendingSearch& ps, const SearchWorkspace& ws, int64_t row0, const Stage& sg, bool first) {
@@ -322,6 +358,14 @@
     W.extra.perm_mod = (int)plan.perm_mod;
     W.extra.row_bound = (int)ix->ntotal;
     const bool track_ovf = ps.nq <= OVF_ROWS;
+    const int64_t n_launches = (ps.nq + MAX_NQ_PER_PASS - 1) / MAX_NQ_PER_PASS * (int64_t)plan.stages.size();
+    const bool stamps = ix->profile && !ix->profile_events && ix->wall_khz > 0 && n_launches <= FILTER_STAMP_SLOTS;
+    ix->enq_stamps = stamps ? (int)n_launches : 0;
+    ix->enq_stages = (int)plan.stages.size();
+    int launch = 0;
+    const StatusOut closing = (ps.defer_flags || ps.band) ? StatusOut() : status_out(ix, ps.slot, ix->enq_stamps);
+    bool published = false;
+    if (closing.host) ix->overflow_host[SLOT_WORDS * ps.slot] = 0;
     const SearchWorkspace& ws = W;
     for (int64_t qb = 0; qb < ps.nq; qb += MAX_NQ_PER_PASS) {
         const int64_t nq = std::min(MAX_NQ_PER_PASS, ps.nq - qb);
@@ -337,7 +381,8 @@
         W.extra.q_map = q_map;
         for (size_t c = 0; c < plan.stages.size(); ++c) {
             const Stage& sg = plan.stages[c];
-            if (launch_stage(ix, W, plan, sg, nq, nq_pad, experiment, stream)) return -1;
+            if (launch_stage(ix, W, plan, sg, nq, nq_pad, experiment, stream, stamps ? launch : -1)) return -1;
+            ++launch;
             if (ps.band) {
                 HIP_OK(launch_exact_rescore(exact_stage_args(ix, ps, ws, row0, sg, c == 0), nq, stream));
                 continue;
@@ -349,13 +394,16 @@
                 dense_n = sg.n_groups;
                 flags |= 2;
             }
-            HIP_OK(launch_select(ws, nq, k, dense_n, flags, stream, ps.id_base, ps.out_scores + row0 * k, ps.out_ids + row0 * k, q_map));
+            const bool closes = (flags & 1) && qb + MAX_NQ_PER_PASS >= ps.nq && closing.host != nullptr;
+            HIP_OK(launch_select(ws, nq, k, dense_n, flags, stream, ps.id_base, ps.out_scores + row0 * k, ps.out_ids + row0 * k, q_map,
+                                 closes ? closing : StatusOut()));
+            published |= closes;
         }
         if (plan.stages.empty())
             HIP_OK(launch_output(ws, nq, k, ps.id_base, ps.out_scores + qb * k, ps.out_ids + qb * k, stream));
     }
     if (ps.defer_flags) return 0;
-    HIP_OK(hipMemcpyAsync(ix->overflow_host + FLAG_WORDS * ps.slot, ws.overflow, FLAG_WORDS * sizeof(unsigned int), hipMemcpyDeviceToHost, stream));
+    if (!published && enqueue_status_copy(ix, ps.slot, ps.lane, ix->enq_stamps, stream)) return -1;
     HIP_OK(hipEventRecord(ix->done[ps.slot], stream));
     return 0;
 }
@@ -410,8 +458,10 @@
     xa.eps = ix->x_eps + (size_t)ps.slot * OVF_ROWS;
     xa.flag_word = ix->ws_lane[ps.lane].overflow + 1;
     xa.flag_q = ix->x_flag_q + (size_t)ps.slot * OVF_ROWS;
+    xa.status = ix->ws_lane[ps.lane].overflow;
+    xa.status_out = status_out(ix, ps.slot, ix->enq_stamps);
     HIP_OK(launch_exact_rescore(xa, ps.nq, stream));
-    HIP_OK(hipMemcpyAsync(ix->overflow_host + FLAG_WORDS * ps.slot, ix->ws_lane[ps.lane].overflow, FLAG_WORDS * sizeof(unsigned int), hipMemcpyDeviceToHost, stream));
+    if (!xa.status_out.host && enqueue_status_copy(ix, ps.slot, ps.lane, ix->enq_stamps, stream)) return -1;
     HIP_OK(hipEventRecord(ix->done[ps.slot], stream));
     return 0;
 }
@@ -447,8 +497,9 @@
     return 0;
 }
 
-int enqueue_l2_finish(vodhip_index* ix, const PendingSearch& ps, hipStream_t stream) {
-    HIP_OK(launch_l2_finish(ix->l2_sim[ps.slot], ix->l2_qn[ps.slot], ps.nq, ps.k, ps.l2_out, stream));
+int enqueue_l2_finish(vodhip_index* ix, const PendingSearch& ps, hipStream_t stream, bool closes = false) {
+    HIP_OK(launch_l2_finish(ix->l2_sim[ps.slot], ix->l2_qn[ps.slot], ps.nq, ps.k, ps.l2_out, stream, ix->ws_lane[ps.lane].overflow,
+                            closes ? status_out(ix, ps.slot, ix->enq_stamps) : StatusOut()));
     return 0;
 }
 
@@ -482,6 +533,9 @@
     ix->exact = exact;
     if (hipDeviceGetAttribute(&ix->tune.n_cu, hipDeviceAttributeMultiprocessorCount, device) != hipSuccess || ix->tune.n_cu < 1) ix->tune.n_cu = 256;
     ix->ws_lane[0].n_cu = ix->ws_lane[1].n_cu = ix->tune.n_cu;
+    int wall_khz = 0;
+    if (hipDeviceGetAttribute(&wall_khz, hipDeviceAttributeWallClockRate, device) != hipSuccess) (void)hipGetLastError();
+    ix->wall_khz = wall_khz > 0 ? wall_khz : 0;
     const size_t bytes = (size_t)ix->capacity_pad * ix->dim_pad * 2;
     hipError_t e = hipMalloc((void**)&ix->data, bytes);
     if (e != hipSuccess) {
@@ -492,7 +546,11 @@
     if (e == hipSuccess) e = hipStreamSynchronize(nullptr);
     if (e == hipSuccess) e = hipMalloc((void**)&ix->ovf_q, MAX_IN_FLIGHT * OVF_ROWS * sizeof(unsigned int));
     if (e == hipSuccess) e = hipMalloc((void**)&ix->q_map, MAX_IN_FLIGHT * OVF_ROWS * sizeof(int));
-    if (e == hipSuccess) e = hipHostMalloc((void**)&ix->overflow_host, FLAG_WORDS * MAX_IN_FLIGHT * sizeof(unsigned int), hipHostMallocDefault);
+    if (e == hipSuccess) e = hipHostMalloc((void**)&ix->overflow_host, SLOT_WORDS * MAX_IN_FLIGHT * sizeof(unsigned int), hipHostMallocMapped | hipHostMallocCoherent);
+    if (e == hipSuccess && hipHostGetDevicePointer((void**)&ix->overflow_host_dev, ix->overflow_host, 0) != hipSuccess) {
+        (void)hipGetLastError();
+        ix->overflow_host_dev = nullptr;
+    }
     for (int i = 0; i < MAX_IN_FLIGHT && e == hipSuccess; ++i) e = hipEventCreateWithFlags(&ix->done[i], hipEventDisableTiming);
     for (int i = 0; i < MAX_IN_FLIGHT && e == hipSuccess; ++i) e = hipEventCreateWithFlags(&ix->lane_in[i], hipEventDisableTiming);
     if (e == hipSuccess) e = hipStreamCreateWithFlags(&ix->lane_stream, hipStreamNonBlocking);
@@ -527,7 +585,7 @@
         delete ix;
         return fail("store initialisation failed: %s", hipGetErrorString(e));
     }
-    for (int i = 0; i < FLAG_WORDS * MAX_IN_FLIGHT; ++i) ix->overflow_host[i] = 0;
+    for (int i = 0; i < SLOT_WORDS * MAX_IN_FLIGHT; ++i) ix->overflow_host[i] = 0;
     *out = ix;
     return 0;
 }
@@ -817,10 +875,10 @@
         ps.out_scores = ix->l2_sim[ps.slot];
         PendingSearch first = ps;
         first.defer_flags = true;
+        if (ix->overflow_host_dev) ix->overflow_host[SLOT_WORDS * ps.slot] = 0;
         if (enqueue_search(ix, first, ix->force_safe != 0, 0, stream)) return -1;
-        const SearchWorkspace& ws = ix->ws_lane[ps.lane];
-        if (l2_profile_mark(ix, ps.slot, 2, stream) || enqueue_l2_finish(ix, ps, stream) || l2_profile_mark(ix, ps.slot, 3, stream) ||
-            hipMemcpyAsync(ix->overflow_host + FLAG_WORDS * ps.slot, ws.overflow, FLAG_WORDS * sizeof(unsigned int), hipMemcpyDeviceToHost, stream) != hipSuccess ||
+        if (l2_profile_mark(ix, ps.slot, 2, stream) || enqueue_l2_finish(ix, ps, stream, true) || l2_profile_mark(ix, ps.slot, 3, stream) ||
+            (!ix->overflow_host_dev && enqueue_status_copy(ix, ps.slot, ps.lane, ix->enq_stamps, stream)) ||
             hipEventRecord(ix->done[ps.slot], stream) != hipSuccess) {
             (void)hipGetLastError();
             (void)hipStreamSynchronize(stream);
@@ -843,17 +901,34 @@
         return -1;
     }
     ps.ev_end = ix->ev_used;
+    if (nq > 0) {
+        ps.n_stamps = ix->enq_stamps;
+        ps.n_stages = ix->enq_stages;
+    }
     ix->next_slot = (ix->next_slot + 1) % MAX_IN_FLIGHT;
     ix->inflight.push_back(ps);
     return 0;
 }
 
 namespace {
+
+int account_recovery(vodhip_index* ix, int slot, size_t ev_first) {
+    read_stamps(ix, slot, ix->enq_stamps, 0, &ix->last_recovery_ns, nullptr);
+    ix->last_recovery_launches += ix->enq_stamps;
+    for (size_t e = ev_first; e + 1 < ix->ev_used; e += 2) {
+        float ms = 0.f;
+        HIP_OK(hipEventElapsedTime(&ms, ix->ev_pool[e], ix->ev_pool[e + 1]));
+        ix->last_recovery_ns += (int64_t)((double)ms * 1e6);
+        ++ix->last_recovery_launches;
+    }
+    ix->ev_used = ev_first;
+    return 0;
+}
 
 int recover_overflow(vodhip_index* ix, const PendingSearch& ps, hipStream_t stream) {
     PendingSearch rs = ps;
     int pass = 0;
-    while (ix->overflow_host[FLAG_WORDS * ps.slot]) {
+    while (ix->overflow_host[SLOT_WORDS * ps.slot]) {
         if (++pass > 40) return fail("internal error: the exhaustive schedule overflowed");
         ix->last_overflow = 1;
         ix->last_safe_reruns += 1;
@@ -874,13 +949,7 @@
         const size_t ev_first = ix->ev_used;
         if (enqueue_search(ix, rs, false, pass + (ps.band ? 1 : 0), stream)) return -1;
         HIP_OK(hipStreamSynchronize(stream));
-        for (size_t e = ev_first; e + 1 < ix->ev_used; e += 2) {
-            float ms = 0.f;
-            HIP_OK(hipEventElapsedTime(&ms, ix->ev_pool[e], ix->ev_pool[e + 1]));
-            ix->last_recovery_ns += (int64_t)((double)ms * 1e6);
-            ++ix->last_recovery_launches;
-        }
-        ix->ev_used = ev_first;
+        if (account_recovery(ix, ps.slot, ev_first)) return -1;
     }
     return pass;
 }
@@ -912,10 +981,14 @@
     ix->last_exact_kx = ps.kx;
     ix->last_exact_band_queries = 0;
     ix->last_exact_band_passes = 0;
-    ix->last_exact_need = ps.kx > 0 && ps.nq > 0 ? (int64_t)ix->overflow_host[FLAG_WORDS * ps.slot + 2] : 0;
-    ix->last_ring_fallbacks = ps.nq > 0 ? (int64_t)ix->overflow_host[FLAG_WORDS * ps.slot + 3] : 0;
+    ix->last_exact_need = ps.kx > 0 && ps.nq > 0 ? (int64_t)ix->overflow_host[SLOT_WORDS * ps.slot + 2] : 0;
+    ix->last_ring_fallbacks = ps.nq > 0 ? (int64_t)ix->overflow_host[SLOT_WORDS * ps.slot + 3] : 0;
+    std::fill(ix->last_stage_ns, ix->last_stage_ns + STAGE_STATS, 0);
+    ix->last_filter_launches = ps.n_stamps;
+    ix->last_filter_ns = 0;
+    read_stamps(ix, ps.slot, ps.n_stamps, ps.n_stages, &ix->last_filter_ns, ix->last_stage_ns);
     if (ps.kx > 0 && ps.nq > 0 && ix->exact_adapt && ix->exact_expand_x100 == 0) {
-        const int need = (int)ix->overflow_host[FLAG_WORDS * ps.slot + 2];
+        const int need = (int)ix->overflow_host[SLOT_WORDS * ps.slot + 2];
         const int formula = exact_kx(ix, ps.k), limit = exact_kx(ix, ps.k, true);
         int target = need >= ps.kx ? std::min(limit, (ps.kx + ps.kx / 4 + 7) / 8 * 8) : std::min(limit, (need + need / 16 + 8 + 7) / 8 * 8);
         target = std::max(target, std::min(formula, ps.k + 8));
@@ -938,7 +1011,7 @@
             if (enqueue_exact_list(ix, ps, stream)) return -1;
             HIP_OK(hipStreamSynchronize(stream));
         }
-        if (ix->overflow_host[FLAG_WORDS * ps.slot + 1]) {
+        if (ix->overflow_host[SLOT_WORDS * ps.slot + 1]) {
             std::vector<unsigned int> flags((size_t)ps.nq);
             HIP_OK(hipMemcpy(flags.data(), ix->x_flag_q + (size_t)ps.slot * OVF_ROWS, (size_t)ps.nq * sizeof(unsigned int), hipMemcpyDeviceToHost));
             std::vector<int> rows;
@@ -958,13 +1031,7 @@
                 const size_t ev_first = ix->ev_used;
                 if (enqueue_search(ix, bs, false, 1, stream)) return -1;
                 HIP_OK(hipStreamSynchronize(stream));
-                for (size_t e = ev_first; e + 1 < ix->ev_used; e += 2) {
-                    float ms = 0.f;
-                    HIP_OK(hipEventElapsedTime(&ms, ix->ev_pool[e], ix->ev_pool[e + 1]));
-                    ix->last_recovery_ns += (int64_t)((double)ms * 1e6);
-                    ++ix->last_recovery_launches;
-                }
-                ix->ev_used = ev_first;
+                if (account_recovery(ix, ps.slot, ev_first)) return -1;
                 const int more = recover_overflow(ix, bs, stream);
                 if (more < 0) return -1;
                 ix->last_exact_band_passes = 1 + more;
@@ -979,12 +1046,13 @@
         HIP_OK(hipEventElapsedTime(&ms, ix->l2_ev[ps.slot][2], ix->l2_ev[ps.slot][3]));
         ix->last_l2_finish_ns = (int64_t)((double)ms * 1e6);
     }
-    ix->last_filter_launches = (int64_t)((ps.ev_end - ps.ev_begin) / 2);
-    ix->last_filter_ns = 0;
+    ix->last_filter_launches += (int64_t)((ps.ev_end - ps.ev_begin) / 2);
     for (size_t e = ps.ev_begin; e + 1 < ps.ev_end; e += 2) {
         float ms = 0.f;
         HIP_OK(hipEventElapsedTime(&ms, ix->ev_pool[e], ix->ev_pool[e + 1]));
-        ix->last_filter_ns += (int64_t)((double)ms * 1e6);
+        const int64_t ns = (int64_t)((double)ms * 1e6);
+        ix->last_filter_ns += ns;
+        if (ps.n_stages > 0) ix->last_stage_ns[std::min<size_t>(((e - ps.ev_begin) / 2) % (size_t)ps.n_stages, STAGE_STATS - 1)] += ns;
     }
     return 0;
 }
@@ -1443,6 +1511,13 @@
     return 0;
 }
 
+int vodhip_debug_stamp_ns(uint64_t start_ticks, uint64_t end_ticks, int64_t rate_khz, int64_t* ns) {
+    if (!ns) return fail("ns is NULL");
+    const int64_t v = filter_stamp_ns(start_ticks, end_ticks, rate_khz);
+    *ns = v < 0 ? 0 : v;
+    return v < 0 ? 0 : 1;
+}
+
 int vodhip_index_set_param(vodhip_index_t* ix, const char* key, int64_t value) {
     if (!ix || !key) return fail("NULL argument");
     if (!strcmp(key, "cand_cap")) {
@@ -1464,6 +1539,9 @@
         ix->tune.sample_div = value;
     } else if (!strcmp(key, "profile")) {
         ix->profile = value;
+    } else if (!strcmp(key, "profile_events")) {
+        if (value < 0 || value > 1) return fail("profile_events must be 0 (in-kernel stamps) or 1 (HIP events around every filter launch)");
+        ix->profile_events = value;
     } else if (!strcmp(key, "ingest_threads")) {
         if (value < 0 || value > 256) return fail("ingest_threads must be in [0, 256] (0 = auto)");
         ix->ingest_threads = value;
@@ -1514,7 +1592,12 @@
         *out = ix->last_filter_launches;
     else if (!strcmp(key, "last_filter_ns"))
         *out = ix->last_filter_ns;
-    else if (!strcmp(key, "last_recovery_launches"))
+    else if (!strncmp(key, "last_stage_ns_", 14)) {
+        char* end = nullptr;
+        const long st = strtol(key + 14, &end, 10);
+        if (end == key + 14 || *end != '\0' || st < 0) return fail("unknown stat '%s'", key);
+        *out = st < STAGE_STATS ? ix->last_stage_ns[st] : 0;
+    } else if (!strcmp(key, "last_recovery_launches"))
         *out = ix->last_recovery_launches;
     else if (!strcmp(key, "last_recovery_ns"))
         *out = ix->last_recovery_ns;
diff --git a/vod_amd/csrc/vodhip_internal.h b/vod_amd/csrc/vodhip_internal.h
--- a/vod_amd/csrc/vodhip_internal.h
+++ b/vod_amd/csrc/vodhip_internal.h
@@ -49,7 +49,26 @@
     int sample_groups = 0;
     const int* q_map = nullptr;
     int perm_mul = 0, perm_mod = 0, row_bound = 0;
-};
+    int stamp_slot = -1;
+};
+
+constexpr int FILTER_FLAG_WORDS = 4;
+constexpr int FILTER_STAMP_SLOTS = 63;
+constexpr int FILTER_STATUS_WORDS = FILTER_FLAG_WORDS + 4 * FILTER_STAMP_SLOTS;
+constexpr int FILTER_TICKET_WORD = FILTER_STATUS_WORDS;
+constexpr int FILTER_WORKSPACE_WORDS = FILTER_STATUS_WORDS + 4;
+
+struct StatusOut {
+    unsigned int* host = nullptr;
+    int n_words = 0;
+};
+
+inline int64_t filter_stamp_ns(uint64_t start, uint64_t end, int64_t rate_khz) {
+    if (rate_khz <= 0) return -1;
+    if (start == ~0ull || end < start) return 0;
+    const uint64_t d = end - start, r = (uint64_t)rate_khz;
+    return (int64_t)(d / r * 1000000u + d % r * 1000000u / r);
+}
 
 struct SearchWorkspace {
     uint16_t* q_pad = nullptr;
@@ -78,7 +97,8 @@
                                  const float* seed_scores, const int64_t* seed_ids, int k, const int* q_map, hipStream_t stream,
                                  const float* seed_margin = nullptr);
 hipError_t launch_select(const SearchWorkspace& ws, int64_t nq, int k, int64_t dense_n, int flags, hipStream_t stream,
-                         int64_t id_base = 0, float* out_scores = nullptr, int64_t* out_ids = nullptr, const int* q_map = nullptr);
+                         int64_t id_base = 0, float* out_scores = nullptr, int64_t* out_ids = nullptr, const int* q_map = nullptr,
+                         StatusOut status_out = StatusOut());
 hipError_t launch_output(const SearchWorkspace& ws, int64_t nq, int k, int64_t id_base, float* out_scores,
                          int64_t* out_ids, hipStream_t stream);
 hipError_t launch_merge_topk(const float* scores, const int64_t* ids, int64_t stride_s, int64_t stride_i, int n_shards,
@@ -133,6 +153,8 @@
     float* eps = nullptr;
     unsigned int* flag_word = nullptr;
     unsigned int* flag_q = nullptr;
+    unsigned int* status = nullptr;
+    StatusOut status_out;
 };
 constexpr int EXACT_MAX_OUTLIERS = 32;
 enum : int { EXS_MAX_N2 = 0, EXS_MAX_D2 = 1, EXS_ORD_N2 = 2, EXS_ORD_D2 = 3, EXS_N_OUT = 4, EXS_CUT_N2 = 5, EXS_CUT_D2 = 6,
@@ -175,7 +197,8 @@
                           hipStream_t stream);
 hipError_t launch_l2_stage_queries(const void* q_src, int q_dtype, int64_t nq, int64_t dim, int store_dtype, void* staged, float* qn,
                                    hipStream_t stream);
-hipError_t launch_l2_finish(const float* sim, const float* qn, int64_t nq, int k, float* dist, hipStream_t stream);
+hipError_t launch_l2_finish(const float* sim, const float* qn, int64_t nq, int k, float* dist, hipStream_t stream,
+                            const unsigned int* status = nullptr, StatusOut status_out = StatusOut());
 
 struct ScanInputs {
     const void* store = nullptr;
```

Result: no change. 81500 queries/s (median of 6 runs) (+0.4%).
